# sndels/yuki

Measured on AMD Instinct MI355X. Metric: Mray/s (primary+secondary), Path integrator @1080p, higher is better.
Workload: dtype f32; 1 GPU; cfg3: city 40x20 displaced icospheres, 1,024,012 triangles, SAH BVH (max_shapes_in_node 1), Path 8 bounces, Stratified 8x8, 1920x1080; triangles=1024012, spp=64, max_depth=8, tiles=8160, partition=single GPU, frames_in_flight=2

## Files before the change

### include/yuki_hip.h

```cpp
#ifndef YUKI_HIP_H
#define YUKI_HIP_H
#include <stddef.h>
#include <stdint.h>

#ifdef __cplusplus
extern "C" {
#endif

#define YK_ABI_VERSION 1

typedef enum yk_status {
    YK_OK = 0,
    YK_ERR_INVALID_ARGUMENT = 1,
    YK_ERR_NO_DEVICE = 2,
    YK_ERR_DEVICE = 3,
    YK_ERR_OUT_OF_MEMORY = 4,
    YK_ERR_UNSUPPORTED = 5,
    YK_ERR_BVH_BUILD = 6,
    YK_ERR_CANCELLED = 7,
    YK_ERR_STACK_OVERFLOW = 8
} yk_status;


typedef struct yk_mesh_desc {
// ... 136 lines not shown
    uint32_t builder;
    uint32_t reason;
    uint32_t levels;
    uint32_t small_range;
    uint64_t small_ranges;
    double seconds_upload;
    double seconds_levels;
    double seconds_small;
    double seconds_layout;
    double seconds_copy_back;
} yk_bvh_build_info;

typedef struct yk_render_stats {
    uint64_t rays;
    uint64_t shadow_rays;
    uint64_t samples;
    double seconds_total;
    double seconds_trace;
    double seconds_shadow;
    double seconds_shade;
    uint32_t trace_launches, batches;
    uint32_t shadow_launches, reserved;
} yk_render_stats;

typedef struct yk_context yk_context;
typedef struct yk_scene yk_scene;

typedef int (*yk_cancel_fn)(void* user);

uint32_t yk_abi_version(void);
const char* yk_status_string(yk_status s);
yk_status yk_context_create(int device, yk_context** out);
void yk_context_destroy(yk_context* ctx);
yk_status yk_last_error(const yk_context* ctx, char* buf, size_t cap);
void* yk_context_stream(const yk_context* ctx);
yk_status yk_context_interrupt(yk_context* ctx);
yk_status yk_context_set_option(yk_context* ctx, const char* key, int64_t value);

yk_status yk_camera_init(const yk_camera_params* params, yk_camera* out);
size_t yk_film_tiles(uint16_t res_x, uint16_t res_y, uint16_t tile_dim, yk_tile* out, size_t cap);
yk_status yk_make_rect_light(const float light_to_world[16], const float light_to_world_inv[16], const float radiance[3],
                             const float size[2], yk_light_desc* out);
yk_status yk_make_spot_light(const float light_to_world[16], const float light_to_world_inv[16], const float intensity[3],
                             float total_width_degrees, float falloff_start_degrees, yk_light_desc* out);
yk_status yk_make_point_light(const float light_to_world[16], const float intensity[3], yk_light_desc* out);
yk_status yk_film_update_tiles(const yk_tile* tiles, size_t n_tiles, const float* tile_rgb, uint16_t res_x, uint16_t res_y,
                               float* film_rgb);

yk_status yk_scene_create(yk_context* ctx, const yk_scene_desc* desc, yk_scene** out);
yk_status yk_scene_create_device(yk_context* ctx, const yk_scene_desc* desc, void* stream, yk_scene** out);
yk_status yk_scene_update(yk_context* ctx, yk_scene* scene, const float* points, const float* normals);
yk_status yk_scene_update_device(yk_context* ctx, yk_scene* scene, const float* d_points, const float* d_normals, void* stream);
enum { YK_UPDATE_ROUTE_HOST = 0, YK_UPDATE_ROUTE_DEVICE = 1 };
typedef struct yk_scene_update_info {
    uint32_t n_updates;
    uint32_t route;
    uint32_t reason;
    uint32_t n_levels;
    uint64_t plan_bytes;
    double seconds_check, seconds_boxes, seconds_records, seconds_total;
} yk_scene_update_info;
yk_status yk_scene_get_update_info(const yk_scene* scene, yk_scene_update_info* out);
yk_status yk_bvh_refit(yk_bvh_node* nodes, size_t n_nodes, const uint32_t* shape_order, size_t n_shapes, const float* shape_bounds);
void yk_scene_destroy(yk_scene* scene);
yk_status yk_scene_get_info(const yk_scene* scene, yk_scene_info* out);
yk_status yk_scene_export_bvh(const yk_scene* scene, yk_bvh_node* nodes, uint32_t* shape_order);
yk_status yk_scene_get_build_info(const yk_scene* scene, yk_bvh_build_info* out);
enum { YK_LAYOUT_HOST = 0, YK_LAYOUT_DEVICE = 1 };
enum {
    YK_LAYOUT_REASON_NONE = 0,
    YK_LAYOUT_REASON_OUT_OF_MEMORY = 1,
    YK_LAYOUT_REASON_DEVICE_ERROR = 2,
    YK_LAYOUT_REASON_MULTI = 3
};
typedef struct yk_scene_layout_info {
    uint32_t layout;
    uint32_t reason;
    double seconds_upload;
    double seconds_layout;
    uint32_t tree_fetched;
    uint32_t root_ref, n_top, n_top_any, wide, wide_auto;
} yk_scene_layout_info;
yk_status yk_scene_get_layout_info(const yk_scene* scene, yk_scene_layout_info* out);
enum { YK_RECORDS_NODES = 0, YK_RECORDS_NODES4 = 1, YK_RECORDS_TOP = 2, YK_RECORDS_TOP_ANY = 3, YK_RECORDS_TRIS = 4, YK_RECORDS_PRIM_SHADE = 5, YK_RECORDS_PRIM_ATTR = 6 };
yk_status yk_scene_read_records(const yk_scene* scene, uint32_t which, void* out, size_t cap_bytes, size_t* n_bytes);
size_t yk_layout_top_order(const yk_bvh_node* nodes, size_t n, uint32_t cap, uint32_t* out_order);
size_t yk_layout_wide_slots(const yk_bvh_node* nodes, size_t n, uint32_t* out_slot_per_node);
size_t yk_bvh_partition_plan(const uint8_t* pass, size_t n, uint32_t* order);

yk_status yk_render_tiles(yk_context* ctx, const yk_scene* scene, const yk_camera* camera, const yk_sampler_desc* sampler,
                          const yk_integrator_desc* integrator, const yk_tile* tiles, size_t n_tiles, float* out_rgb,
                          yk_render_stats* stats, yk_cancel_fn cancel, void* user);
yk_status yk_render_tiles_device(yk_context* ctx, const yk_scene* scene, const yk_camera* camera,
                                 const yk_sampler_desc* sampler, const yk_integrator_desc* integrator, const yk_tile* tiles,
                                 size_t n_tiles, void* d_out_rgb, void* stream, yk_render_stats* stats, yk_cancel_fn cancel,
                                 void* user);
yk_status yk_render_tiles_accumulating(yk_context* ctx, const yk_scene* scene, const yk_camera* camera, const yk_sampler_desc* sampler,
                                       const yk_integrator_desc* integrator, const yk_tile* tiles, const uint16_t* tile_samples, size_t n_tiles,
                                       float* out_rgb, yk_render_stats* stats, yk_cancel_fn cancel, void* user);
yk_status yk_render_tiles_accumulating_device(yk_context* ctx, const yk_scene* scene, const yk_camera* camera, const yk_sampler_desc* sampler,
                                              const yk_integrator_desc* integrator, const yk_tile* tiles, const uint16_t* tile_samples,
                                              size_t n_tiles, void* d_out_rgb, void* stream, yk_render_stats* stats, yk_cancel_fn cancel,
                                              void* user);
yk_status yk_film_accumulate_tiles(const yk_tile* tiles, size_t n_tiles, const float* tile_rgb, uint16_t res_x, uint16_t res_y, float* film_rgb,
                                   uint32_t* tile_sample_counts);
yk_status yk_film_accumulate_tiles_device(yk_context* ctx, const yk_tile* tiles, size_t n_tiles, const void* d_tile_rgb, uint16_t res_x,
                                          uint16_t res_y, void* d_film_rgb, void* stream);
typedef struct yk_tile_list yk_tile_list;
yk_status yk_tile_list_create(yk_context* ctx, const yk_tile* tiles, const uint16_t* tile_samples, size_t n_tiles, yk_tile_list** out);
void yk_tile_list_destroy(yk_tile_list* list);
yk_status yk_render_tile_list_device(yk_context* ctx, const yk_scene* scene, const yk_camera* camera, const yk_sampler_desc* sampler,
                                     const yk_integrator_desc* integrator, const yk_tile_list* list, void* d_out_rgb, void* stream,
                                     yk_render_stats* stats, yk_cancel_fn cancel, void* user);
yk_status yk_film_update_tile_list_device(yk_context* ctx, const yk_tile_list* list, const void* d_tile_rgb, uint16_t res_x, uint16_t res_y,
                                          void* d_film_rgb, void* stream, int accumulate);
yk_status yk_render_tiles_accumulating_passes(yk_context* ctx, const yk_scene* scene, const yk_camera* camera, const yk_sampler_desc* sampler,
                                              const yk_integrator_desc* integrator, const yk_tile* tiles, const uint16_t* tile_samples,
                                              size_t n_tiles, uint32_t n_passes, float* out_rgb, yk_render_stats* stats, yk_cancel_fn cancel,
                                              void* user);
yk_status yk_render_tile_list_passes_device(yk_context* ctx, const yk_scene* scene, const yk_camera* camera, const yk_sampler_desc* sampler,
                                            const yk_integrator_desc* integrator, const yk_tile_list* list, uint32_t n_passes, void* d_out_rgb,
                                            void* stream, yk_render_stats* stats, yk_cancel_fn cancel, void* user);
yk_status yk_render_tile_list_samples_device(yk_context* ctx, const yk_scene* scene, const yk_camera* camera, const yk_sampler_desc* sampler,
                                             const yk_integrator_desc* integrator, const yk_tile_list* list, uint32_t first_sample,
                                             uint32_t n_passes, void* d_out_rgb, void* stream, yk_render_stats* stats, yk_cancel_fn cancel,
                                             void* user);
yk_status yk_film_accumulate_tile_list_passes_device(yk_context* ctx, const yk_tile_list* list, const void* d_passes_rgb, uint32_t n_passes,
                                                     uint16_t res_x, uint16_t res_y, void* d_film_rgb, void* stream);

yk_status yk_write_exr(const char* path, uint32_t width, uint32_t height, const float* rgb);
yk_status yk_write_pfm(const char* path, uint32_t width, uint32_t height, const float* rgb);

typedef enum yk_tone_map_kind { YK_TONE_MAP_RAW = 0, YK_TONE_MAP_FILMIC = 1, YK_TONE_MAP_HEATMAP = 2 } yk_tone_map_kind;
typedef enum yk_heatmap_channel { YK_HEATMAP_RED = 0, YK_HEATMAP_GREEN = 1, YK_HEATMAP_BLUE = 2, YK_HEATMAP_LUMINANCE = 3 } yk_heatmap_channel;
typedef struct yk_tone_map_desc {
    uint32_t kind;
    float exposure;
    uint32_t channel;
    uint32_t has_bounds;
    float bounds[2];
} yk_tone_map_desc;
yk_status yk_tone_map(yk_context* ctx, const yk_tone_map_desc* desc, const float* film_rgb, uint16_t res_x, uint16_t res_y,
                      uint16_t tile_dim, const uint32_t* samples, float* out_rgb, float* used_bounds);
yk_status yk_tone_map_device(yk_context* ctx, const yk_tone_map_desc* desc, const void* d_film_rgb, uint16_t res_x, uint16_t res_y,
                             uint16_t tile_dim, const uint32_t* samples, void* d_out_rgb, void* stream);
yk_status yk_film_min_max(yk_context* ctx, const float* film_rgb, uint16_t res_x, uint16_t res_y, uint32_t channel, float out_min_max[2]);

typedef struct yk_exposure_desc {
    uint32_t low_cut, high_cut;
    float ev_bias, min_ev, max_ev, adapt_up, adapt_down;
    uint16_t window[4];
} yk_exposure_desc;
typedef struct yk_exposure_state {
    float exposure, log2_adapted, log2_metered;
    uint32_t frames, counted, skipped, below, above;
} yk_exposure_state;
yk_status yk_film_histogram(yk_context* ctx, const float* film_rgb, uint16_t res_x, uint16_t res_y, uint16_t tile_dim, const uint32_t* samples,
                            const uint16_t window[4], uint32_t out_bins[256], uint32_t out_skipped_below_above[3]);
yk_status yk_exposure_meter(yk_context* ctx, const yk_exposure_desc* desc, const float* film_rgb, uint16_t res_x, uint16_t res_y, uint16_t tile_dim,
                            const uint32_t* samples, const yk_exposure_state* prev, yk_exposure_state* out);
yk_status yk_exposure_meter_device(yk_context* ctx, const yk_exposure_desc* desc, const void* d_film_rgb, uint16_t res_x, uint16_t res_y,
                                   uint16_t tile_dim, const uint32_t* samples, const void* d_prev, void* d_out_state, void* stream);
yk_status yk_tone_map_metered_device(yk_context* ctx, const yk_tone_map_desc* desc, const void* d_state, const void* d_film_rgb, uint16_t res_x,
                                     uint16_t res_y, uint16_t tile_dim, const uint32_t* samples, void* d_out_rgb, void* stream);

yk_status yk_render_tile(yk_context* ctx, const yk_scene* scene, const yk_camera* camera, const yk_sampler_desc* sampler,
                         const yk_integrator_desc* integrator, const yk_tile* tile, float* tile_pixels, uint64_t* out_rays);
yk_status yk_film_update_tiles_device(yk_context* ctx, const yk_tile* tiles, size_t n_tiles, const void* d_tile_rgb,
// ... 296 lines not shown
```

### yuki_amd/_ffi.py

```python
import ctypes as C
import os
import subprocess

from . import abi

_HERE = os.path.dirname(os.path.abspath(__file__))
LIB_PATH = os.environ.get("YK_LIB_PATH") or os.path.join(_HERE, "libyuki_hip.so")
_LIB = None

YK_OK = 0
STATUS_NAMES = {
    0: "YK_OK",
    1: "YK_ERR_INVALID_ARGUMENT",
    2: "YK_ERR_NO_DEVICE",
    3: "YK_ERR_DEVICE",
    4: "YK_ERR_OUT_OF_MEMORY",
    5: "YK_ERR_UNSUPPORTED",
    6: "YK_ERR_BVH_BUILD",
    7: "YK_ERR_CANCELLED",
    8: "YK_ERR_STACK_OVERFLOW",
}


class YukiError(RuntimeError):
# ... 6 lines not shown
    _fields_ = [
        ("n_nodes", C.c_uint64),
        ("n_interior", C.c_uint64),
        ("n_shapes", C.c_uint64),
        ("bounds_min", C.c_float * 3),
        ("bounds_max", C.c_float * 3),
        ("build_seconds", C.c_double),
        ("upload_seconds", C.c_double),
        ("device_bytes", C.c_uint64),
        ("max_leaf_shapes", C.c_uint32),
        ("tree_depth", C.c_uint32),
    ]


class BvhBuildInfo(C.Structure):
    _fields_ = [
        ("builder", C.c_uint32),
        ("reason", C.c_uint32),
        ("levels", C.c_uint32),
        ("small_range", C.c_uint32),
        ("small_ranges", C.c_uint64),
        ("seconds_upload", C.c_double),
        ("seconds_levels", C.c_double),
        ("seconds_small", C.c_double),
        ("seconds_layout", C.c_double),
        ("seconds_copy_back", C.c_double),
    ]


BVH_BUILDER_NAMES = {0: "host recursion", 1: "device", 2: "host levels"}
BVH_REASON_NAMES = {0: "", 1: "split method", 2: "non-finite bound", 3: "select_nth on a long range", 4: "too many nodes", 5: "out of device memory", 6: "device error"}


class RenderStats(C.Structure):
    _fields_ = [
        ("rays", C.c_uint64),
        ("shadow_rays", C.c_uint64),
        ("samples", C.c_uint64),
        ("seconds_total", C.c_double),
        ("seconds_trace", C.c_double),
        ("seconds_shadow", C.c_double),
        ("seconds_shade", C.c_double),
        ("trace_launches", C.c_uint32),
        ("batches", C.c_uint32),
        ("shadow_launches", C.c_uint32),
        ("reserved", C.c_uint32),
    ]


class CombinerInfo(C.Structure):
    _fields_ = [("submissions", C.c_uint64), ("tiles", C.c_uint64), ("requeued", C.c_uint64), ("largest_submission", C.c_uint32), ("lanes", C.c_uint32)]


CANCEL_FN = C.CFUNCTYPE(C.c_int, C.c_void_p)

vp = C.c_void_p
SYMBOLS = {
    "yk_abi_version": (C.c_uint32, []),
    "yk_status_string": (C.c_char_p, [C.c_int]),
    "yk_context_create": (C.c_int, [C.c_int, C.POINTER(vp)]),
    "yk_context_destroy": (None, [vp]),
    "yk_last_error": (C.c_int, [vp, C.c_char_p, C.c_size_t]),
    "yk_context_stream": (vp, [vp]),
    "yk_context_set_option": (C.c_int, [vp, C.c_char_p, C.c_int64]),
    "yk_camera_init": (C.c_int, [C.POINTER(abi.CameraParams), C.POINTER(abi.CameraMatrices)]),
    "yk_film_tiles": (C.c_size_t, [C.c_uint16, C.c_uint16, C.c_uint16, vp, C.c_size_t]),
    "yk_make_rect_light": (C.c_int, [abi.f32p, abi.f32p, abi.f32p, abi.f32p, C.POINTER(abi.LightDesc)]),
    "yk_make_spot_light": (C.c_int, [abi.f32p, abi.f32p, abi.f32p, C.c_float, C.c_float, C.POINTER(abi.LightDesc)]),
    "yk_make_point_light": (C.c_int, [abi.f32p, abi.f32p, C.POINTER(abi.LightDesc)]),
    "yk_film_update_tiles": (C.c_int, [vp, C.c_size_t, vp, C.c_uint16, C.c_uint16, vp]),
    "yk_scene_create": (C.c_int, [vp, C.POINTER(abi.SceneDesc), C.POINTER(vp)]),
    "yk_scene_create_device": (C.c_int, [vp, C.POINTER(abi.SceneDesc), vp, C.POINTER(vp)]),
    "yk_scene_update": (C.c_int, [vp, vp, vp, vp]),
    "yk_scene_update_device": (C.c_int, [vp, vp, vp, vp, vp]),
    "yk_scene_get_update_info": (C.c_int, [vp, C.POINTER(abi.SceneUpdateInfo)]),
    "yk_bvh_refit": (C.c_int, [vp, C.c_size_t, vp, C.c_size_t, vp]),
    "yk_scene_destroy": (None, [vp]),
    "yk_scene_get_info": (C.c_int, [vp, C.POINTER(SceneInfo)]),
    "yk_scene_export_bvh": (C.c_int, [vp, vp, vp]),
    "yk_scene_get_build_info": (C.c_int, [vp, C.POINTER(BvhBuildInfo)]),
    "yk_bvh_partition_plan": (C.c_size_t, [vp, C.c_size_t, vp]),
    "yk_scene_get_layout_info": (C.c_int, [vp, C.POINTER(abi.SceneLayoutInfo)]),
    "yk_scene_read_records": (C.c_int, [vp, C.c_uint32, vp, C.c_size_t, C.POINTER(C.c_size_t)]),
    "yk_layout_top_order": (C.c_size_t, [vp, C.c_size_t, C.c_uint32, vp]),
    "yk_layout_wide_slots": (C.c_size_t, [vp, C.c_size_t, vp]),
    "yk_render_tiles": (C.c_int, [vp, vp, C.POINTER(abi.CameraMatrices), C.POINTER(abi.SamplerDesc), C.POINTER(abi.IntegratorDesc), vp, C.c_size_t, vp, C.POINTER(RenderStats), vp, vp]),
    "yk_render_tiles_device": (C.c_int, [vp, vp, C.POINTER(abi.CameraMatrices), C.POINTER(abi.SamplerDesc), C.POINTER(abi.IntegratorDesc), vp, C.c_size_t, vp, vp, C.POINTER(RenderStats), vp, vp]),
    "yk_render_tile": (C.c_int, [vp, vp, C.POINTER(abi.CameraMatrices), C.POINTER(abi.SamplerDesc), C.POINTER(abi.IntegratorDesc), C.POINTER(abi.Tile), vp, C.POINTER(C.c_uint64)]),
    "yk_film_update_tiles_device": (C.c_int, [vp, vp, C.c_size_t, vp, C.c_uint16, C.c_uint16, vp, vp]),
    "yk_li": (C.c_int, [vp, vp, C.POINTER(abi.SamplerDesc), C.POINTER(abi.IntegratorDesc), C.c_size_t, vp, vp, vp, vp, C.c_uint32, vp, vp]),
    "yk_li_debug": (C.c_int, [vp, vp, C.POINTER(abi.SamplerDesc), C.POINTER(abi.IntegratorDesc), C.c_size_t, vp, vp, vp, vp, C.c_uint32, C.c_uint32, vp, vp, vp, vp]),
    "yk_trace_closest": (C.c_int, [vp, vp, C.c_size_t] + [vp] * 9),
    "yk_trace_any": (C.c_int, [vp, vp, C.c_size_t] + [vp] * 5),
    "yk_sampler_sequence": (C.c_int, [vp, C.POINTER(abi.SamplerDesc), C.c_uint16, C.c_uint16, C.c_uint32, vp, C.c_size_t, vp]),
    "yk_camera_rays": (C.c_int, [vp, C.POINTER(abi.CameraMatrices), C.POINTER(abi.SamplerDesc), C.POINTER(abi.Tile), C.c_uint32, vp, vp]),
    "yk_device_math": (C.c_int, [vp, C.c_int, C.c_size_t, vp, vp, vp]),
    "yk_host_math": (C.c_int, [C.c_int, C.c_size_t, vp, vp, vp]),
    "yk_bsdf_eval": (C.c_int, [vp, C.POINTER(abi.MaterialDesc), C.c_size_t] + [vp] * 6),
    "yk_bsdf_sample": (C.c_int, [vp, C.POINTER(abi.MaterialDesc), C.c_size_t] + [vp] * 6),
    "yk_light_sample": (C.c_int, [vp, C.POINTER(abi.LightDesc), C.c_int32, C.c_size_t] + [vp] * 4),
    "yk_sizeof": (C.c_size_t, [C.c_int]),
    "yk_load_ply": (C.c_int, [C.c_char_p, C.c_uint32, C.c_uint32, C.POINTER(vp)]),
    "yk_load_pbrt": (C.c_int, [C.c_char_p, C.c_uint32, C.c_uint32, C.POINTER(vp)]),
    "yk_load_mitsuba": (C.c_int, [C.c_char_p, C.c_uint32, C.c_uint32, C.POINTER(vp)]),
    "yk_load_scene": (C.c_int, [C.c_char_p, C.c_uint32, C.c_uint32, C.POINTER(vp)]),
    "yk_loaded_scene_get": (C.c_int, [vp, C.POINTER(abi.SceneDesc), C.POINTER(abi.CameraParams), C.POINTER(C.c_uint16)]),
    "yk_loaded_scene_destroy": (None, [vp]),
    "yk_loader_last_error": (C.c_char_p, []),
    "yk_image_texture_load": (C.c_int, [C.c_char_p, C.POINTER(abi.TextureDesc)]),
    "yk_image_texture_free": (None, [C.POINTER(abi.TextureDesc)]),
    "yk_render_tiles_accumulating": (C.c_int, [vp, vp, C.POINTER(abi.CameraMatrices), C.POINTER(abi.SamplerDesc), C.POINTER(abi.IntegratorDesc), vp, vp, C.c_size_t, vp, C.POINTER(RenderStats), vp, vp]),
    "yk_render_tiles_accumulating_device": (C.c_int, [vp, vp, C.POINTER(abi.CameraMatrices), C.POINTER(abi.SamplerDesc), C.POINTER(abi.IntegratorDesc), vp, vp, C.c_size_t, vp, vp, C.POINTER(RenderStats), vp, vp]),
    "yk_film_accumulate_tiles": (C.c_int, [vp, C.c_size_t, vp, C.c_uint16, C.c_uint16, vp, vp]),
    "yk_film_accumulate_tiles_device": (C.c_int, [vp, vp, C.c_size_t, vp, C.c_uint16, C.c_uint16, vp, vp]),
    "yk_tile_list_create": (C.c_int, [vp, vp, vp, C.c_size_t, C.POINTER(vp)]),
    "yk_tile_list_destroy": (None, [vp]),
    "yk_render_tile_list_device": (C.c_int, [vp, vp, C.POINTER(abi.CameraMatrices), C.POINTER(abi.SamplerDesc), C.POINTER(abi.IntegratorDesc), vp, vp, vp, C.POINTER(RenderStats), vp, vp]),
    "yk_film_update_tile_list_device": (C.c_int, [vp, vp, vp, C.c_uint16, C.c_uint16, vp, vp, C.c_int]),
    "yk_render_tiles_accumulating_passes": (C.c_int, [vp, vp, C.POINTER(abi.CameraMatrices), C.POINTER(abi.SamplerDesc), C.POINTER(abi.IntegratorDesc), vp, vp, C.c_size_t, C.c_uint32, vp, C.POINTER(RenderStats), vp, vp]),
    "yk_render_tile_list_samples_device": (C.c_int, [vp, vp, C.POINTER(abi.CameraMatrices), C.POINTER(abi.SamplerDesc), C.POINTER(abi.IntegratorDesc), vp, C.c_uint32, C.c_uint32, vp, vp, C.POINTER(RenderStats), vp, vp]),
    "yk_render_tile_list_passes_device": (C.c_int, [vp, vp, C.POINTER(abi.CameraMatrices), C.POINTER(abi.SamplerDesc), C.POINTER(abi.IntegratorDesc), vp, C.c_uint32, vp, vp, C.POINTER(RenderStats), vp, vp]),
    "yk_film_accumulate_tile_list_passes_device": (C.c_int, [vp, vp, vp, C.c_uint32, C.c_uint16, C.c_uint16, vp, vp]),
    "yk_write_exr": (C.c_int, [C.c_char_p, C.c_uint32, C.c_uint32, vp]),
    "yk_write_pfm": (C.c_int, [C.c_char_p, C.c_uint32, C.c_uint32, vp]),
    "yk_tone_map": (C.c_int, [vp, C.POINTER(abi.ToneMapDesc), vp, C.c_uint16, C.c_uint16, C.c_uint16, vp, vp, vp]),
    "yk_tone_map_device": (C.c_int, [vp, C.POINTER(abi.ToneMapDesc), vp, C.c_uint16, C.c_uint16, C.c_uint16, vp, vp, vp]),
    "yk_film_min_max": (C.c_int, [vp, vp, C.c_uint16, C.c_uint16, C.c_uint32, vp]),
    "yk_film_histogram": (C.c_int, [vp, vp, C.c_uint16, C.c_uint16, C.c_uint16, vp, vp, vp, vp]),
    "yk_exposure_meter": (C.c_int, [vp, C.POINTER(abi.ExposureDesc), vp, C.c_uint16, C.c_uint16, C.c_uint16, vp, C.POINTER(abi.ExposureState), C.POINTER(abi.ExposureState)]),
    "yk_exposure_meter_device": (C.c_int, [vp, C.POINTER(abi.ExposureDesc), vp, C.c_uint16, C.c_uint16, C.c_uint16, vp, vp, vp, vp]),
    "yk_tone_map_metered_device": (C.c_int, [vp, C.POINTER(abi.ToneMapDesc), vp, vp, C.c_uint16, C.c_uint16, C.c_uint16, vp, vp, vp]),
    "yk_scene_node_bounds": (C.c_size_t, [vp, C.c_int32, vp, C.c_size_t]),
    "yk_overlay_world_to_clip": (C.c_int, [C.POINTER(abi.CameraParams), vp, vp]),
    "yk_overlay_ray_lines": (C.c_int, [vp, C.c_size_t, vp]),
    "yk_overlay_draw": (C.c_int, [vp, vp, vp, C.c_size_t, vp, C.c_size_t, vp, C.c_uint16, C.c_uint16]),
    "yk_overlay_draw_device": (C.c_int, [vp, vp, vp, C.c_size_t, vp, C.c_size_t, vp, C.c_uint16, C.c_uint16, vp]),
    "yk_present_target_rect": (C.c_int, [C.c_uint16, C.c_uint16, C.c_uint16, C.c_uint16, C.POINTER(abi.PresentRect)]),
    "yk_present": (C.c_int, [vp, C.POINTER(abi.PresentDesc), vp, C.c_uint16, C.c_uint16, vp]),
    "yk_present_device": (C.c_int, [vp, C.POINTER(abi.PresentDesc), vp, C.c_uint16, C.c_uint16, vp, vp]),
    "yk_render_guides": (C.c_int, [vp, vp, C.POINTER(abi.CameraMatrices), C.c_uint16, C.c_uint16, vp]),
    "yk_render_guides_device": (C.c_int, [vp, vp, C.POINTER(abi.CameraMatrices), C.c_uint16, C.c_uint16, vp, vp]),
    "yk_denoise": (C.c_int, [vp, C.POINTER(abi.DenoiseDesc), vp, vp, C.c_uint16, C.c_uint16, C.c_uint16, vp, vp]),
    "yk_denoise_device": (C.c_int, [vp, C.POINTER(abi.DenoiseDesc), vp, vp, C.c_uint16, C.c_uint16, C.c_uint16, vp, vp, vp]),
    "yk_history_reproject": (C.c_int, [vp, C.POINTER(abi.TemporalDesc), vp, vp, C.POINTER(abi.CameraMatrices), vp, C.c_uint16, C.c_uint16, vp]),
    "yk_history_reproject_device": (C.c_int, [vp, C.POINTER(abi.TemporalDesc), vp, vp, C.POINTER(abi.CameraMatrices), vp, C.c_uint16, C.c_uint16, vp, vp]),
    "yk_history_blend": (C.c_int, [vp, C.POINTER(abi.TemporalDesc), vp, C.c_uint16, C.c_uint16, C.c_uint16, vp, vp, vp, vp]),
    "yk_history_blend_device": (C.c_int, [vp, C.POINTER(abi.TemporalDesc), vp, C.c_uint16, C.c_uint16, C.c_uint16, vp, vp, vp, vp, vp]),
    "yk_render_guides_ids": (C.c_int, [vp, vp, C.POINTER(abi.CameraMatrices), C.c_uint16, C.c_uint16, vp, vp]),
    "yk_render_guides_ids_device": (C.c_int, [vp, vp, C.POINTER(abi.CameraMatrices), C.c_uint16, C.c_uint16, vp, vp, vp]),
    "yk_surface_motion": (C.c_int, [vp, vp, vp, vp, vp, C.c_uint16, C.c_uint16, vp]),
    "yk_surface_motion_device": (C.c_int, [vp, vp, vp, vp, vp, C.c_uint16, C.c_uint16, vp, vp]),
    "yk_surface_albedo": (C.c_int, [vp, vp, vp, C.c_uint16, C.c_uint16, vp]),
    "yk_surface_albedo_device": (C.c_int, [vp, vp, vp, C.c_uint16, C.c_uint16, vp, vp]),
    "yk_albedo_mean": (C.c_int, [vp, vp, vp, C.c_uint16, C.c_uint16, C.c_uint32, vp]),
    "yk_albedo_mean_device": (C.c_int, [vp, vp, vp, C.c_uint16, C.c_uint16, C.c_uint32, vp, vp]),
    "yk_render_albedo_mean": (C.c_int, [vp, vp, C.POINTER(abi.CameraMatrices), C.c_uint16, C.c_uint16, C.c_uint32, vp]),
    "yk_render_albedo_mean_device": (C.c_int, [vp, vp, C.POINTER(abi.CameraMatrices), C.c_uint16, C.c_uint16, C.c_uint32, vp, vp]),
    "yk_denoise_albedo": (C.c_int, [vp, C.POINTER(abi.DenoiseDesc), vp, vp, vp, C.c_uint16, C.c_uint16, C.c_uint16, vp, vp]),
    "yk_denoise_albedo_device": (C.c_int, [vp, C.POINTER(abi.DenoiseDesc), vp, vp, vp, C.c_uint16, C.c_uint16, C.c_uint16, vp, vp, vp]),
    "yk_history_reproject_moved": (C.c_int, [vp, C.POINTER(abi.TemporalDesc), vp, vp, C.POINTER(abi.CameraMatrices), vp, vp, C.c_uint16, C.c_uint16, vp]),
    "yk_history_reproject_moved_device": (C.c_int, [vp, C.POINTER(abi.TemporalDesc), vp, vp, C.POINTER(abi.CameraMatrices), vp, vp, C.c_uint16, C.c_uint16, vp, vp]),
    "yk_moments_blend": (C.c_int, [vp, C.POINTER(abi.TemporalDesc), vp, C.c_uint16, C.c_uint16, C.c_uint16, vp, vp, vp]),
    "yk_moments_blend_device": (C.c_int, [vp, C.POINTER(abi.TemporalDesc), vp, C.c_uint16, C.c_uint16, C.c_uint16, vp, vp, vp, vp]),
    "yk_variance": (C.c_int, [vp, C.POINTER(abi.VarianceDesc), vp, vp, vp, vp, C.c_uint16, C.c_uint16, C.c_uint16, vp, vp]),
    "yk_variance_device": (C.c_int, [vp, C.POINTER(abi.VarianceDesc), vp, vp, vp, vp, C.c_uint16, C.c_uint16, C.c_uint16, vp, vp, vp]),
    "yk_denoise_variance": (C.c_int, [vp, C.POINTER(abi.VarianceDesc), vp, vp, vp, vp, C.c_uint16, C.c_uint16, C.c_uint16, vp, vp]),
# ... 79 lines not shown
```

### yuki_amd/abi.py

```python
import ctypes as C

import numpy as np

f32p = C.POINTER(C.c_float)
u32p = C.POINTER(C.c_uint32)
i32p = C.POINTER(C.c_int32)


class MeshDesc(C.Structure):
    _fields_ = [("has_normals", C.c_uint8), ("has_uvs", C.c_uint8), ("swaps_handedness", C.c_uint8), ("pad", C.c_uint8)]


class SphereDesc(C.Structure):
    _fields_ = [
        ("object_to_world", C.c_float * 16),
        ("world_to_object", C.c_float * 16),
        ("radius", C.c_float),
        ("material", C.c_int32),
    ]


class MaterialDesc(C.Structure):
    _fields_ = [("kind", C.c_uint32), ("a", C.c_float * 3), ("b", C.c_float * 3), ("c", C.c_float), ("flags", C.c_uint32), ("a_texture", C.c_uint32)]

# ... 156 lines not shown
    _fields_ = [
        ("bmin", C.c_float * 3),
        ("bmax", C.c_float * 3),
        ("a", C.c_uint32),
        ("count", C.c_uint16),
        ("axis", C.c_uint8),
        ("is_leaf", C.c_uint8),
    ]


class SceneLayoutInfo(C.Structure):

    _fields_ = [
        ("layout", C.c_uint32),
        ("reason", C.c_uint32),
        ("seconds_upload", C.c_double),
        ("seconds_layout", C.c_double),
        ("tree_fetched", C.c_uint32),
        ("root_ref", C.c_uint32),
        ("n_top", C.c_uint32),
        ("n_top_any", C.c_uint32),
        ("wide", C.c_uint32),
        ("wide_auto", C.c_uint32),
    ]


class SceneUpdateInfo(C.Structure):

    _fields_ = [
        ("n_updates", C.c_uint32),
        ("route", C.c_uint32),
        ("reason", C.c_uint32),
        ("n_levels", C.c_uint32),
        ("plan_bytes", C.c_uint64),
        ("seconds_check", C.c_double),
        ("seconds_boxes", C.c_double),
        ("seconds_records", C.c_double),
        ("seconds_total", C.c_double),
    ]


class TraceStats(C.Structure):
    _fields_ = [
        ("closest_rays", C.c_uint64),
        ("closest_node_tests", C.c_uint64),
        ("closest_shape_tests", C.c_uint64),
        ("shadow_rays", C.c_uint64),
        ("shadow_node_tests", C.c_uint64),
        ("shadow_shape_tests", C.c_uint64),
    ]


BVH_NODE_DTYPE = np.dtype(
    [("bmin", "<f4", 3), ("bmax", "<f4", 3), ("a", "<u4"), ("count", "<u2"), ("axis", "u1"), ("is_leaf", "u1")]
)
TILE_DTYPE = np.dtype([("x0", "<u2"), ("y0", "<u2"), ("x1", "<u2"), ("y1", "<u2")])
INTEGRATOR_RAY_DTYPE = np.dtype([("o", "<f4", 3), ("d", "<f4", 3), ("t_max", "<f4"), ("ray_type", "<u4")])
OVERLAY_LINE_DTYPE = np.dtype([("p0", "<f4", 3), ("p1", "<f4", 3), ("rgb", "<f4", 3)])
GUIDE_DTYPE = np.dtype([("ns", "<f4", 3), ("hit", "<f4"), ("p", "<f4", 3), ("t", "<f4")])
HISTORY_DTYPE = np.dtype([("rgb", "<f4", 3), ("n", "<f4")])
SURFACE_NONE = 0xFFFFFFFF
SURFACE_ID_DTYPE = np.dtype([("shape", "<u4"), ("b", "<f4", 3)])
MOTION_DTYPE = np.dtype([("p_prev", "<f4", 3), ("known", "<f4")])
ALBEDO_DTYPE = np.dtype([("a", "<f4", 3), ("known", "<f4")])
ALBEDO_FLOOR = 0.015625
ALBEDO_MEAN_MAX_S = 8
MOMENTS_DTYPE = np.dtype([("m1", "<f4"), ("m2", "<f4"), ("frames", "<f4"), ("n", "<f4")])
PIXEL_STATS_DTYPE = np.dtype([("mean", "<f4"), ("m2", "<f4"), ("n", "<u4"), ("drawn", "<u4")])

SPLIT_SAH, SPLIT_MIDDLE, SPLIT_EQUAL_COUNTS = 0, 1, 2
MAT_MATTE, MAT_GLASS, MAT_METAL, MAT_GLOSSY = 0, 1, 2, 3
LIGHT_POINT, LIGHT_SPOT, LIGHT_DISTANT, LIGHT_RECT = 0, 1, 2, 3
SAMPLER_UNIFORM, SAMPLER_STRATIFIED = 0, 1
INTEGRATOR_WHITTED, INTEGRATOR_PATH, INTEGRATOR_BVH_INTERSECTIONS, INTEGRATOR_GEOMETRY_NORMALS, INTEGRATOR_SHADING_NORMALS, INTEGRATOR_SHADING_UVS = 0, 1, 2, 3, 4, 5
RAY_DIRECT, RAY_REFLECTION, RAY_REFRACTION, RAY_NORMAL, RAY_SHADOW = 0, 1, 2, 3, 4
FOV_X, FOV_Y = 0, 1
TONE_MAP_RAW, TONE_MAP_FILMIC, TONE_MAP_HEATMAP = 0, 1, 2
HEATMAP_RED, HEATMAP_GREEN, HEATMAP_BLUE, HEATMAP_LUMINANCE = 0, 1, 2, 3
PRESENT_ENCODE_NONE, PRESENT_ENCODE_SHADER, PRESENT_ENCODE_SRGB = 0, 1, 2
PRESENT_RGBA8, PRESENT_RGB32F = 0, 1
LAYOUT_HOST, LAYOUT_DEVICE = 0, 1
UPDATE_ROUTE_HOST, UPDATE_ROUTE_DEVICE = 0, 1
LAYOUT_REASON_NONE, LAYOUT_REASON_OUT_OF_MEMORY, LAYOUT_REASON_DEVICE_ERROR, LAYOUT_REASON_MULTI = 0, 1, 2, 3
RECORDS_NODES, RECORDS_NODES4, RECORDS_TOP, RECORDS_TOP_ANY, RECORDS_TRIS, RECORDS_PRIM_SHADE, RECORDS_PRIM_ATTR = range(7)
RECORD_NAMES = ("nodes", "nodes4", "top", "top_any", "tris", "prim_shade", "prim_attr")


def ptr(a, ty):
    if a is None:
        return C.cast(None, ty)
    assert a.flags["C_CONTIGUOUS"]
    return a.ctypes.data_as(ty)


def f3(v):
    return (C.c_float * 3)(*[float(x) for x in v])


def f16(m):
    return (C.c_float * 16)(*[float(x) for x in np.asarray(m, dtype=np.float32).reshape(16)])
```

### yuki_amd/core.py

```python
import ctypes as C
from dataclasses import dataclass

import numpy as np

from . import _ffi, abi
from ._ffi import BvhBuildInfo, RenderStats, SceneInfo, YukiError, check, lib


def _p(a):
    return None if a is None else a.ctypes.data_as(C.c_void_p)


def _vp(a):
    return C.c_void_p(a) if a else None


def _film(film):
    film = np.ascontiguousarray(film, dtype=np.float32)
    if film.ndim != 3 or film.shape[2] != 3:
        raise ValueError("film is (h, w, 3)")
    return film, film.shape[1], film.shape[0]


def _scene_diagonal(scene):
# ... 896 lines not shown

    def reproject_history_moved_device(self, d_prev_history_ptr, d_prev_guides_ptr, prev_camera, d_guides_ptr, d_motion_ptr, res, params, d_out_history_ptr, stream=None):
        d = _temporal_desc(params)
        check(lib().yk_history_reproject_moved_device(self.h, C.byref(d), _vp(d_prev_history_ptr), _vp(d_prev_guides_ptr), C.byref(prev_camera.matrices), _vp(d_guides_ptr), _vp(d_motion_ptr), int(res[0]), int(res[1]), _vp(d_out_history_ptr), _vp(stream)), self.h)

    def blend_history_device(self, d_film_ptr, res, params, tile_dim, samples, d_history_ptr, d_out_history_ptr, d_out_rgb_ptr, stream=None):
        d = _temporal_desc(params)
        samples = _blend_samples(res, tile_dim, samples)
        check(lib().yk_history_blend_device(self.h, C.byref(d), _vp(d_film_ptr), int(res[0]), int(res[1]), int(tile_dim), _p(samples), _vp(d_history_ptr), _vp(d_out_history_ptr), _vp(d_out_rgb_ptr), _vp(stream)), self.h)

    def blend_moments_device(self, d_film_ptr, res, params, tile_dim, samples, d_moments_ptr, d_out_moments_ptr, stream=None):
        d = _temporal_desc(params)
        samples = _blend_samples(res, tile_dim, samples)
        check(lib().yk_moments_blend_device(self.h, C.byref(d), _vp(d_film_ptr), int(res[0]), int(res[1]), int(tile_dim), _p(samples), _vp(d_moments_ptr), _vp(d_out_moments_ptr), _vp(stream)), self.h)

    def variance_device(self, d_moments_ptr, d_film_ptr, d_guides_ptr, res, params, tile_dim, samples, d_out_ptr, stream=None, albedo=None):
        d = _variance_desc(params)
        samples = _blend_samples(res, tile_dim, samples)
        check(lib().yk_variance_device(self.h, C.byref(d), _vp(d_moments_ptr), _vp(d_film_ptr), _vp(d_guides_ptr), _vp(albedo), int(res[0]), int(res[1]), int(tile_dim), _p(samples), _vp(d_out_ptr), _vp(stream)), self.h)

    def denoise_variance_device(self, d_film_ptr, d_guides_ptr, d_variance_ptr, res, params, tile_dim, samples, d_out_ptr, stream=None, albedo=None):
        d = _variance_desc(params)
        samples = _blend_samples(res, tile_dim, samples)
        check(lib().yk_denoise_variance_device(self.h, C.byref(d), _vp(d_film_ptr), _vp(d_guides_ptr), _vp(d_variance_ptr), _vp(albedo), int(res[0]), int(res[1]), int(tile_dim), _p(samples), _vp(d_out_ptr), _vp(stream)), self.h)

    def adaptive_select_device(self, d_stats_ptr, res, params, pixel_list, stream=None):
        d = _adaptive_desc(params)
        n = C.c_uint32(0)
        check(lib().yk_adaptive_select_device(self.h, C.byref(d), _vp(d_stats_ptr), int(res[0]), int(res[1]), pixel_list.h, C.byref(n), _vp(stream)), self.h)
        pixel_list.n = n.value
        return n.value

    def adaptive_accumulate_device(self, pixel_list, d_passes_ptr, n_passes, res, d_film_sum_ptr, d_stats_ptr, stream=None):
        check(lib().yk_adaptive_accumulate_device(self.h, pixel_list.h, _vp(d_passes_ptr), int(n_passes), int(res[0]), int(res[1]), _vp(d_film_sum_ptr), _vp(d_stats_ptr), _vp(stream)), self.h)

    def adaptive_resolve_device(self, d_film_sum_ptr, d_stats_ptr, res, d_out_rgb_ptr, d_out_variance_ptr, stream=None):
        check(lib().yk_adaptive_resolve_device(self.h, _vp(d_film_sum_ptr), _vp(d_stats_ptr), int(res[0]), int(res[1]), _vp(d_out_rgb_ptr), _vp(d_out_variance_ptr), _vp(stream)), self.h)

    @property
    def stream_handle(self):
        return int(lib().yk_context_stream(self.h) or 0)

    def close(self):
        if getattr(self, "h", None):
            lib().yk_context_destroy(self.h)
            self.h = None

    def __del__(self):
        try:
            self.close()
        except Exception:
            pass


def _device_addresses(given, table, ctx, stream):
    address, tensors = {}, []
    for name, (dtypes, expected) in table.items():
        a = given.get(name)
        if a is None or isinstance(a, (int, np.integer)):
            address[name] = int(a) if a else None
            continue
        if not hasattr(a, "data_ptr"):
            raise ValueError(f"{name}: expected a torch tensor or a device address, got {type(a).__name__}")
        if str(a.dtype).replace("torch.", "") not in dtypes:
            raise ValueError(f"{name}: element type {a.dtype}, expected {' or '.join(dtypes)}")
        if not a.is_contiguous():
            raise ValueError(f"{name}: the tensor is not contiguous")
        if a.numel() != expected:
            raise ValueError(f"{name}: {a.numel()} elements, expected {expected}")
        tensors.append((name, a))
    for name, a in tensors:
        if not a.is_cuda or a.device.index != ctx.device:
            raise ValueError(f"{name}: the tensor is on {a.device}, not on the context's device {ctx.device}")
        address[name] = a.data_ptr() or None
    if stream is None and tensors:
        import torch

        torch.cuda.current_stream(tensors[0][1].device).synchronize()
    elif stream is not None and not isinstance(stream, int):
        stream = stream.cuda_stream
    return address, stream


class Scene:

    def __init__(self, ctx, scene_data):
        self.ctx = ctx
        self.data = scene_data
        d, self._keep = scene_data.desc(LightFactory)
        self.n_lights = int(d.n_lights)
        h = C.c_void_p()
        check(lib().yk_scene_create(ctx.h if ctx else None, C.byref(d), C.byref(h)), ctx.h if ctx else None)
        self.h = h
        self._keep = None

    DEVICE_ARRAYS = {
        "points": (abi.f32p, ("float32",), "v", 3),
        "normals": (abi.f32p, ("float32",), "v", 3),
        "uvs": (abi.f32p, ("float32",), "v", 2),
        "indices": (abi.u32p, ("uint32", "int32"), "t", 3),
        "tri_mesh": (abi.u32p, ("uint32", "int32"), "t", 1),
        "tri_material": (abi.i32p, ("int32",), "t", 1),
        "tri_area_light": (abi.i32p, ("int32",), "t", 1),
        "shape_order": (abi.u32p, ("uint32", "int32"), "s", 1),
    }

    @classmethod
    def from_device(cls, ctx, scene_data, arrays, stream=None):
        unknown = set(arrays) - set(cls.DEVICE_ARRAYS)
        if unknown:
            raise ValueError(f"unknown device arrays {sorted(unknown)}; the names are {sorted(cls.DEVICE_ARRAYS)}")
        counts = {"v": int(scene_data.points.shape[0]), "t": int(scene_data.indices.shape[0])}
        counts["s"] = counts["t"] + len(scene_data.spheres)
        address, stream = _device_addresses(arrays, {name: (dtypes, k * counts[per]) for name, (_, dtypes, per, k) in cls.DEVICE_ARRAYS.items()}, ctx, stream)
        self = cls.__new__(cls)
        self.ctx, self.data = ctx, scene_data
        d, keep = scene_data.desc(LightFactory)
        for name, (ptype, _, _, _) in cls.DEVICE_ARRAYS.items():
            setattr(d, name, C.cast(C.c_void_p(address[name]), ptype))
        self.n_lights = int(d.n_lights)
        h = C.c_void_p()
        check(lib().yk_scene_create_device(ctx.h, C.byref(d), _vp(stream), C.byref(h)), ctx.h)
        self.h = h
        del keep
        return self

    def close(self):
        if getattr(self, "h", None):
            lib().yk_scene_destroy(self.h)
            self.h = None

    def __del__(self):
        try:
            self.close()
        except Exception:
            pass

    def info(self):
        i = SceneInfo()
        check(lib().yk_scene_get_info(self.h, C.byref(i)))
        return i

    def build_info(self):
        i = BvhBuildInfo()
        check(lib().yk_scene_get_build_info(self.h, C.byref(i)))
        return i

    def layout_info(self):
        i = abi.SceneLayoutInfo()
        check(lib().yk_scene_get_layout_info(self.h, C.byref(i)))
        return i

    def update(self, points, normals=None, stream=None):
        nv = int(self.data.points.shape[0])
        given = {"points": points, "normals": normals}
        if all(a is None or isinstance(a, np.ndarray) or isinstance(a, (list, tuple)) for a in given.values()):
            host = {}
            for name, a in given.items():
                if a is None:
                    host[name] = None
                    continue
                a = np.ascontiguousarray(a, dtype=np.float32)
                if a.size != 3 * nv:
                    raise ValueError(f"{name}: {a.size} elements, expected {3 * nv}")
                host[name] = a.reshape(nv, 3)
            ctx_h = self.ctx.h if self.ctx else None
# ... 488 lines not shown
```

### yuki_amd/csrc/yk_context.cpp

```cpp
#include <hip/hip_runtime.h>

#include <algorithm>
#include <chrono>
#include <cstdio>
#include <cstdlib>
#include <cstring>
#include <mutex>
#include <string>
#include <vector>

#include "yk_internal.h"

extern "C" {

uint32_t yk_abi_version(void) { return YK_ABI_VERSION; }

const char* yk_status_string(yk_status s) {
    switch (s) {
        case YK_OK: return "ok";
        case YK_ERR_INVALID_ARGUMENT: return "invalid argument";
        case YK_ERR_NO_DEVICE: return "no HIP device";
        case YK_ERR_DEVICE: return "HIP error";
        case YK_ERR_OUT_OF_MEMORY: return "out of device memory";
        case YK_ERR_UNSUPPORTED: return "unsupported on the device path";
// ... 75 lines not shown
    if (ctx->ws[1].stream) (void)hipStreamDestroy(ctx->ws[1].stream);
    if (ctx->ev_in) (void)hipEventDestroy(ctx->ev_in);
    if (ctx->ev_out) (void)hipEventDestroy(ctx->ev_out);
    DevBuf* all[] = {&ctx->sample_buf, &ctx->pixel_xy, &ctx->pixel_aux, &ctx->tiles, &ctx->tile_off, &ctx->counters, &ctx->stats4, &ctx->hit4,
                     &ctx->tile_sample, &ctx->pixel_sample, &ctx->film_tiles, &ctx->film_tile_off, &ctx->film_pixel_xy};
    for (DevBuf* b : all) b->release();
    for (DevBuf& b : ctx->scratch) b.release();
    ctx->tonemap.partials.release();
    ctx->tonemap.bounds.release();
    ctx->tonemap.samples.release();
    ctx->overlay.ids.release();
    ctx->denoise.ping[0].release();
    ctx->denoise.ping[1].release();
    ctx->denoise.samples.release();
    ctx->temporal.samples.release();
    ctx->adaptive.rank.release();
    ctx->adaptive.tile_count.release();
    ctx->albedo_mean.ids_band.release();
    ctx->exposure.slot.release();
    ctx->exposure.samples.release();
    if (ctx->tonemap.staging) (void)hipHostFree(ctx->tonemap.staging);
    if (ctx->tonemap.staged) (void)hipEventDestroy(ctx->tonemap.staged);
    for (hipEvent_t e : ctx->ev_pool) (void)hipEventDestroy(e);
    if (ctx->cancel_stream) {
        (void)hipStreamSynchronize(ctx->cancel_stream);
        (void)hipStreamDestroy(ctx->cancel_stream);
    }
    if (ctx->cancel_host) (void)hipHostFree(ctx->cancel_host);
    (void)hipStreamDestroy(ctx->stream);
    delete ctx;
}

yk_status yk_last_error(const yk_context* ctx, char* buf, size_t cap) {
    if (!buf || cap == 0) return YK_ERR_INVALID_ARGUMENT;
    if (!ctx) {
        std::snprintf(buf, cap, "%s", host_last_error().c_str());
        host_last_error().clear();
        return YK_OK;
    }
    std::snprintf(buf, cap, "%s", ctx->last_error.c_str());
    return YK_OK;
}

void* yk_context_stream(const yk_context* ctx) { return ctx ? (void*)ctx->stream : nullptr; }

yk_status yk_context_set_option(yk_context* ctx, const char* key, int64_t value) {
    if (!ctx || !key) return YK_ERR_INVALID_ARGUMENT;
    YK_LOCK(ctx);
    std::string k(key);
    if (k == "batch_paths") {
        if (value < 64 || value > ((int64_t)1 << 29)) return YK_ERR_INVALID_ARGUMENT;
        ctx->batch_paths = value;
    } else if (k == "sample_buf_cap") {
        if (value < (1 << 20)) return YK_ERR_INVALID_ARGUMENT;
        ctx->sample_buf_cap = value;
    } else if (k == "streams") {
        if (value < 1 || value > 2) return YK_ERR_INVALID_ARGUMENT;
        ctx->streams = value;
    } else if (k == "packet_bounces") {
        if (value < 0) return YK_ERR_INVALID_ARGUMENT;
        ctx->packet_bounces = value;
    } else if (k == "packet_shadow_bounces") {
        if (value < 0) return YK_ERR_INVALID_ARGUMENT;
        ctx->packet_shadow_bounces = value;
    } else if (k == "shade_reorder") {
        ctx->shade_reorder = value != 0;
    } else if (k == "overlap_shadow") {
        ctx->overlap_shadow = value != 0;
    } else if (k == "top_nodes") {
        if (value < 0 || value > YK_TOP_MAX) return YK_ERR_INVALID_ARGUMENT;
        ctx->top_nodes = value;
    } else if (k == "wide_bvh") {
        if (value < 0 || value > 2) return YK_ERR_INVALID_ARGUMENT;
        ctx->wide_bvh = value;
    } else if (k == "bvh_builder") {
        if (value < 0 || value > 1) return YK_ERR_INVALID_ARGUMENT;
        ctx->bvh_builder = value;
    } else if (k == "bvh_small_range") {
        if (value < 0 || value > (1 << 20)) return YK_ERR_INVALID_ARGUMENT;
        ctx->bvh_small_range = value;
    } else if (k == "scene_layout") {
        if (value < 0 || value > 1) return YK_ERR_INVALID_ARGUMENT;
        ctx->scene_layout = value;
    } else if (k == "trace_stage_kernel") {
        if (value < 0 || value > 2) return YK_ERR_INVALID_ARGUMENT;
        ctx->trace_stage_kernel = value;
    } else if (k == "overlay_coop_min") {
        if (value < 1 || value > 65536) return YK_ERR_INVALID_ARGUMENT;
        ctx->overlay.coop_min = value;
    } else if (k == "denoise_lds_max_step") {
        if (value < 0 || value > 2) return YK_ERR_INVALID_ARGUMENT;
        ctx->denoise.lds_max_step = value;
    } else if (k == "albedo_mean_band_rows") {
        if (value < 0 || value > 65535) return YK_ERR_INVALID_ARGUMENT;
        ctx->albedo_mean.band_rows = value;
    } else if (k == "exposure_wave_combine") {
        ctx->exposure.wave_combine = value != 0;
    } else if (k == "update_top_block") {
        ctx->update_top_block = value != 0;
    } else if (k == "time_kernels") {
        ctx->time_kernels = value;
    } else {
        return YK_ERR_INVALID_ARGUMENT;
    }
    return YK_OK;
}

yk_status yk_camera_init(const yk_camera_params* params, yk_camera* out) { return camera_init(params, out); }

size_t yk_film_tiles(uint16_t res_x, uint16_t res_y, uint16_t tile_dim, yk_tile* out, size_t cap) try {
    std::vector<yk_tile> t = film_tiles(res_x, res_y, tile_dim);
    if (out)
        for (size_t i = 0; i < t.size() && i < cap; ++i) out[i] = t[i];
    return t.size();
} catch (const std::exception&) {
    return 0;
}

yk_status yk_make_rect_light(const float l2w[16], const float l2w_inv[16], const float radiance[3], const float size[2], yk_light_desc* out) {
    if (!l2w || !l2w_inv || !radiance || !size || !out) return YK_ERR_INVALID_ARGUMENT;
    std::memset(out, 0, sizeof(*out));
    Xf light_to_world = xf_from(l2w, l2w_inv);
    Xf sample_to_light = xf_mul(xf_scale(size[0], 1.0f, size[1]), xf_translation(-0.5f, 0.0f, -0.5f));
    Xf sample_to_world = xf_mul(light_to_world, sample_to_light);
    out->kind = YK_LIGHT_RECT;
    for (int k = 0; k < 3; ++k) out->i[k] = radiance[k];
    std::memcpy(out->sample_to_world, sample_to_world.m, 64);
    std::memcpy(out->sample_to_world_inv, sample_to_world.mi, 64);
    out->area = size[0] * size[1];
    return YK_OK;
}

yk_status yk_make_spot_light(const float l2w[16], const float l2w_inv[16], const float intensity[3], float total_width_degrees,
                             float falloff_start_degrees, yk_light_desc* out) {
    if (!l2w || !l2w_inv || !intensity || !out) return YK_ERR_INVALID_ARGUMENT;
    std::memset(out, 0, sizeof(*out));
    V3 p = xf_point(l2w, V3{0.0f, 0.0f, 0.0f});
    out->kind = YK_LIGHT_SPOT;
    out->p[0] = p.x;
    out->p[1] = p.y;
    out->p[2] = p.z;
    for (int k = 0; k < 3; ++k) out->i[k] = intensity[k];
    out->cos_total_width = det_cosf(total_width_degrees * (YK_PI / 180.0f));
    out->cos_falloff_start = det_cosf(falloff_start_degrees * (YK_PI / 180.0f));
    std::memcpy(out->world_to_light, l2w_inv, 64);
    return YK_OK;
}

yk_status yk_make_point_light(const float l2w[16], const float intensity[3], yk_light_desc* out) {
    if (!l2w || !intensity || !out) return YK_ERR_INVALID_ARGUMENT;
    std::memset(out, 0, sizeof(*out));
    V3 p = xf_point(l2w, V3{0.0f, 0.0f, 0.0f});
    out->kind = YK_LIGHT_POINT;
    out->p[0] = p.x;
    out->p[1] = p.y;
    out->p[2] = p.z;
    for (int k = 0; k < 3; ++k) out->i[k] = intensity[k];
    return YK_OK;
}

yk_status yk_film_update_tiles(const yk_tile* tiles, size_t n_tiles, const float* tile_rgb, uint16_t res_x, uint16_t res_y, float* film_rgb) {
    if (!tiles || !tile_rgb || !film_rgb) return YK_ERR_INVALID_ARGUMENT;
    size_t off = 0;
    for (size_t t = 0; t < n_tiles; ++t) {
        const yk_tile& tl = tiles[t];
        if (tl.x1 > res_x || tl.y1 > res_y || tl.x0 >= tl.x1 || tl.y0 >= tl.y1) return YK_ERR_INVALID_ARGUMENT;
// ... 57 lines not shown
```

### yuki_amd/csrc/yk_device.h

```cpp
#pragma once
#include <hip/hip_runtime.h>
#include <stdint.h>

#include "../../include/yuki_hip.h"
#include "yk_bsdf.h"
#include "yk_rng.h"

namespace yk {

struct DevNode {
    float4 q0, q1, q2;
    uint4 q3;
};
static_assert(sizeof(DevNode) == 64, "DevNode must be 64 bytes");

#define YK_VIS_STRIDE(nl) ((nl) <= 4u ? 4u : (nl))
#define YK_LEAF_BIT 0x80000000u
#define YK_REF_NONE 0xffffffffu
#define YK_AXIS_SHIFT 28
#define YK_AXIS_MASK (3u << YK_AXIS_SHIFT)
#define YK_REF_INDEX_MAX ((1u << YK_AXIS_SHIFT) - 1u)
#define YK_TOP_BIT 0x40000000u
#define YK_TOP_MAX 1023

struct DevNode4 {
    float4 q0, q1, q2, q3, q4, q5;
    uint4 q6, q7;
};
static_assert(sizeof(DevNode4) == 128, "DevNode4 must be 128 bytes");

struct DevLight {
    uint32_t kind;
    float p[3];
    float i[3];
    float cos_total_width, cos_falloff_start;
    float w2l[16];
    float s2w[16];
    float n[3];
    float area;
};

struct DevSphere {
    float o2w[16];
    float w2o[16];
    float radius;
    int material;
    unsigned swaps_handedness;
    unsigned pad;
};

#define YK_PRIM_LAST 1u
#define YK_PRIM_SPHERE 2u
#define YK_PRIM_KIND_SHIFT 4
#define YK_HIT_KIND_SHIFT 28
#define YK_HIT_PRIM_MASK 0x0fffffffu
#define YK_HIT_WORD(prim, pflags) ((int)((prim) | ((((pflags) >> YK_PRIM_KIND_SHIFT) & 7u) << YK_HIT_KIND_SHIFT)))

#define YK_MESH_NORMALS 1u
#define YK_MESH_UVS 2u
#define YK_MESH_SWAPS 4u

struct DevScene {
    const DevNode* nodes;
    const DevNode4* nodes4;
    const DevNode* top_nodes;
    uint32_t n_top;
    const DevNode* top_nodes_any;
    uint32_t n_top_any;
    const float4* tris;
    const uint4* prim_shade;
    const float4* prim_attr;
    const DevSphere* spheres;
    uint32_t n_triangles;
    uint32_t root_ref;
    float root_bmin[3], root_bmax[3];
    const uint32_t* indices;
    const float* points;
    const float* normals;
    const float* uvs;
    const uint32_t* tri_mesh;
    const int32_t* tri_material;
    const int32_t* tri_area_light;
    const uint32_t* mesh_flags;
    const Material* materials;
    const DevLight* lights;
    uint32_t n_lights;
    float background[3];
    const float4* texels;
    const uint4* tex_info;
};

struct DevCamera {
    float c2w[16];
    float r2c[16];
};

struct PathBuffers {
    float4* rayO;
    float4* rayD;
    float4* thru;
    uint4* rngs;
};

#define YK_CTRL_WORDS 1024
#define YK_CTRL_ERR 3
#define YK_CTRL_CANCELLED 2
#define YK_CTRL_CAM_O (YK_CTRL_WORDS + 32)
#define YK_CTRL_ALLOC_WORDS (YK_CTRL_WORDS + 64)
#define YK_CTRL_HEADS 8
#define YK_CTRL_STRIDE 8
#define YK_CTRL_BOUNCE(b) (8 + YK_CTRL_STRIDE * (b))
#define YK_CTRL_SHQ 1
#define YK_CTRL_SHQ2 2
#define YK_CTRL_HEAD 3
#define YK_CTRL_MAX_DEPTH ((YK_CTRL_WORDS - 8) / YK_CTRL_STRIDE - 1)

struct CancelRef {
    const unsigned* host;
    unsigned* dev;
};
#define YK_HEAD_POISON 0xC0000000u

__device__ __forceinline__ bool cancel_raised(const CancelRef& c) { return c.dev && *c.dev != 0u; }
__device__ __forceinline__ bool cancel_relay(const CancelRef& c, unsigned* head) {
    if (!c.host || __hip_atomic_load(c.host, __ATOMIC_RELAXED, __HIP_MEMORY_SCOPE_SYSTEM) == 0u) return false;
    atomicOr(c.dev, 1u);
    atomicMax(head, YK_HEAD_POISON);
    return true;
}

struct RenderParams {
    SamplerCfg sampler;
    uint32_t max_depth;
    uint32_t has_clamp;
    float clamp;
    uint32_t integrator;
    uint32_t spe;
    uint32_t sample_base;
    CancelRef cancel;
};

__device__ __forceinline__ void split_sample_id(uint32_t sid, uint32_t spe, uint32_t& entry, uint32_t& k) {
    if ((spe & (spe - 1u)) == 0u) {
        entry = sid >> (31u - (uint32_t)__clz((int)spe));
        k = sid & (spe - 1u);
    } else {
        entry = sid / spe;
        k = sid % spe;
    }
}

}
```

### yuki_amd/csrc/yk_geom.h

```cpp
#pragma once
#include "yk_device.h"

namespace yk {

struct RayTri {
    int kx, ky, kz;
    float sx, sy, sz;
};
YK_HD RayTri ray_tri_setup(V3 d) {
    RayTri r;
    r.kz = max_dimension(vabs(d));
    r.kx = r.kz < 2 ? r.kz + 1 : 0;
    r.ky = r.kx < 2 ? r.kx + 1 : 0;
    float dx = comp(d, r.kx), dy = comp(d, r.ky), dz = comp(d, r.kz);
    r.sx = -dx / dz;
    r.sy = -dy / dz;
    r.sz = 1.0f / dz;
    return r;
}

struct TriHit {
    float t, b0, b1, b2;
};

// ... 155 lines not shown
    } else {
        float inv_uv_det = 1.0f / uv_det;
        dpdu = (dp02 * duv12y - dp12 * duv02y) * inv_uv_det;
        dpdv = ((-dp02) * duv12x + dp12 * duv02x) * inv_uv_det;
    }
    (void)dpdv;
    Surface s;
    s.p = p0 * h.b0 + p1 * h.b1 + p2 * h.b2;
    s.u = u0x * h.b0 + u1x * h.b1 + u2x * h.b2;
    s.v = u0y * h.b0 + u1y * h.b1 + u2y * h.b2;
    V3 n = normalize(cross(dp02, dp12));
    if (mflags & YK_MESH_SWAPS) n = -n;
    s.n = n;
    s.ns = n;
    s.dpdus = dpdu;
    if (mflags & YK_MESH_NORMALS) {
        V3 n0 = at.n0, n1 = at.n1, n2 = at.n2;
        V3 ns;
        V3 nn = normalize(n0 * h.b0 + n1 * h.b1 + n2 * h.b2);
        if (len_sqr(nn) > 0.0f)
            ns = normalize(nn);
        else
            ns = s.n;
        V3 ss = normalize(dpdu);
        V3 ts = cross(ss, ns);
        if (len_sqr(ts) > 0.0f) {
            ts = normalize(ts);
            ss = cross(ts, ns);
        } else {
            coordinate_system(ns, ss, ts);
        }
        s.ns = normalize(cross(ss, ts));
        s.n = faceforward_n(s.n, s.ns);
        s.dpdus = ss;
    }
    s.material = 0;
    s.area_light = -1;
    return s;
}

YK_HD Surface make_surface_core(const DevScene& sc, V3 p0, V3 p1, V3 p2, uint32_t i0, uint32_t i1, uint32_t i2, uint32_t mflags, const TriHit& h) {
    TriAttr at;
    at.u0x = at.u0y = at.u1x = at.u1y = at.u2x = at.u2y = 0.0f;
    at.n0 = at.n1 = at.n2 = V3{0.0f, 0.0f, 0.0f};
    if (mflags & YK_MESH_UVS) {
        at.u0x = sc.uvs[2 * i0]; at.u0y = sc.uvs[2 * i0 + 1];
        at.u1x = sc.uvs[2 * i1]; at.u1y = sc.uvs[2 * i1 + 1];
        at.u2x = sc.uvs[2 * i2]; at.u2y = sc.uvs[2 * i2 + 1];
    }
    if (mflags & YK_MESH_NORMALS) {
        at.n0 = ld3(sc.normals, i0);
        at.n1 = ld3(sc.normals, i1);
        at.n2 = ld3(sc.normals, i2);
    }
    return make_surface_vals(p0, p1, p2, at, mflags, h);
}

YK_HD Surface make_surface(const DevScene& sc, uint32_t tri, const TriHit& h) {
    uint32_t i0 = sc.indices[3 * tri], i1 = sc.indices[3 * tri + 1], i2 = sc.indices[3 * tri + 2];
    Surface s = make_surface_core(sc, ld3(sc.points, i0), ld3(sc.points, i1), ld3(sc.points, i2), i0, i1, i2, sc.mesh_flags[sc.tri_mesh[tri]], h);
    s.material = sc.tri_material[tri];
    s.area_light = sc.tri_area_light[tri];
    return s;
}

YK_HD Surface hit_surface(const DevScene& sc, uint32_t shape, V3 o, V3 d) {
    if (shape >= sc.n_triangles) {
        const DevSphere& sp = sc.spheres[shape - sc.n_triangles];
        V3 ro, rd;
        float t = 0.0f;
        sphere_hit_t(sp, o, d, __builtin_inff(), t, ro, rd);
        return make_surface_sphere(sp, ro, rd, t, d, sc.texels != nullptr);
    }
    uint32_t i0 = sc.indices[3 * shape], i1 = sc.indices[3 * shape + 1], i2 = sc.indices[3 * shape + 2];
    RayTri rt = ray_tri_setup(d);
    TriHit th = TriHit{0.0f, 0.0f, 0.0f, 0.0f};
    tri_intersect(o, rt, __builtin_inff(), ld3(sc.points, i0), ld3(sc.points, i1), ld3(sc.points, i2), th);
    Surface s = make_surface(sc, shape, th);
    s.wo = -d;
    return s;
}

YK_HD Surface hit_surface_prim(const DevScene& sc, uint32_t prim, V3 o, V3 d, bool want_uv, float* t_out, uint4* id_out) {
    const float4 v0 = sc.tris[3 * prim], v1 = sc.tris[3 * prim + 1], v2 = sc.tris[3 * prim + 2];
    const uint4 ps = sc.prim_shade[prim];
    const uint32_t src = __float_as_uint(v1.w);
    if (__float_as_uint(v2.w) & YK_PRIM_SPHERE) {
        const DevSphere& sp = sc.spheres[src - sc.n_triangles];
        V3 ro, rd;
        float t = 0.0f;
        sphere_hit_t(sp, o, d, __builtin_inff(), t, ro, rd);
        if (t_out) *t_out = t;
        if (id_out) *id_out = make_uint4(src, 0u, 0u, 0u);
        return make_surface_sphere(sp, ro, rd, t, d, want_uv);
    }
    TriAttr at;
    at.u0x = at.u0y = at.u1x = at.u1y = at.u2x = at.u2y = 0.0f;
    at.n0 = at.n1 = at.n2 = V3{0.0f, 0.0f, 0.0f};
    if (sc.prim_attr && (ps.w & (YK_MESH_NORMALS | YK_MESH_UVS))) {
        const float4 a0 = sc.prim_attr[4 * (size_t)prim], a1 = sc.prim_attr[4 * (size_t)prim + 1], a2 = sc.prim_attr[4 * (size_t)prim + 2], a3 = sc.prim_attr[4 * (size_t)prim + 3];
        at.n0 = V3{a0.x, a0.y, a0.z};
        at.n1 = V3{a1.x, a1.y, a1.z};
        at.n2 = V3{a2.x, a2.y, a2.z};
        at.u0x = a0.w; at.u0y = a1.w;
        at.u1x = a2.w; at.u1y = a3.x;
        at.u2x = a3.y; at.u2y = a3.z;
    }
    RayTri rt = ray_tri_setup(d);
    TriHit th = TriHit{0.0f, 0.0f, 0.0f, 0.0f};
    const V3 p0 = V3{v0.x, v0.y, v0.z}, p1 = V3{v1.x, v1.y, v1.z}, p2 = V3{v2.x, v2.y, v2.z};
    tri_intersect(o, rt, __builtin_inff(), p0, p1, p2, th);
    if (t_out) *t_out = th.t;
    if (id_out) *id_out = make_uint4(src, __float_as_uint(th.b0), __float_as_uint(th.b1), __float_as_uint(th.b2));
    Surface s = sc.prim_attr ? make_surface_vals(p0, p1, p2, at, ps.w & 7u, th) : make_surface_core(sc, p0, p1, p2, ps.x, ps.y, ps.z, ps.w & 7u, th);
    s.material = (int)(ps.w >> 6);
    s.area_light = (int)__float_as_uint(v0.w);
    s.wo = -d;
    return s;
}
YK_HD Surface hit_surface_prim(const DevScene& sc, uint32_t prim, V3 o, V3 d, bool want_uv, float* t_out) { return hit_surface_prim(sc, prim, o, d, want_uv, t_out, nullptr); }
YK_HD Surface hit_surface_prim(const DevScene& sc, uint32_t prim, V3 o, V3 d, bool want_uv) { return hit_surface_prim(sc, prim, o, d, want_uv, nullptr, nullptr); }
YK_HD Surface hit_surface_prim(const DevScene& sc, uint32_t prim, V3 o, V3 d) { return hit_surface_prim(sc, prim, o, d, sc.texels != nullptr, nullptr, nullptr); }

YK_HD RGB texture_eval(const DevScene& sc, unsigned tex, float u, float v) {
    const uint4 info = sc.tex_info[tex];
    float sx = u - truncf(u);
    if (sx < 0.0f) sx = 1.0f + sx;
    float sy = v - truncf(v);
    if (sy < 0.0f) sy = 1.0f + sy;
    sy = 1.0f - sy;
    float fx = sx * (float)info.y - 0.5f;
    float fy = sy * (float)info.z - 0.5f;
    unsigned ix = fx > 0.0f ? (unsigned)fminf(fx, 4.0e9f) : 0u;
    unsigned iy = fy > 0.0f ? (unsigned)fminf(fy, 4.0e9f) : 0u;
    size_t idx = (size_t)iy * info.y + ix;
    const size_t last = (size_t)info.y * info.z - 1;
    if (idx > last) idx = last;
    float4 t = sc.texels[(size_t)info.x + idx];
    return RGB{t.x, t.y, t.z};
}

YK_HD V3 spawn_origin(V3 p, V3 n, V3 d) {
    V3 offset = n * 0.001f;
    return dot(d, n) > 0.0f ? p + offset : p - offset;
}

struct LightSample {
    V3 l;
    RGB li;
    float pdf;
    bool has_vis;
    V3 p1;
    int area_light;
};

YK_HD LightSample sample_light(const DevLight& L, int index, V3 sp, float ux, float uy) {
    LightSample s;
    s.has_vis = true;
    s.area_light = -1;
    s.pdf = 1.0f;
    V3 lp = V3{L.p[0], L.p[1], L.p[2]};
    RGB li = RGB{L.i[0], L.i[1], L.i[2]};
    if (L.kind == YK_LIGHT_POINT) {
        V3 to_light = lp - sp;
        float dist_sqr = len_sqr(to_light);
        s.li = li / dist_sqr;
        float dist = sqrtf(dist_sqr);
        s.l = to_light / dist;
        s.p1 = lp;
    } else if (L.kind == YK_LIGHT_SPOT) {
        V3 to_light = lp - sp;
        float dist_sqr = len_sqr(to_light);
        float dist = sqrtf(dist_sqr);
        s.l = to_light / dist;
        V3 dir_local = normalize(xf_vector(L.w2l, -s.l));
        float ct = dir_local.z;
        float falloff;
        if (ct < L.cos_total_width)
            falloff = 0.0f;
        else if (ct > L.cos_falloff_start)
            falloff = 1.0f;
        else {
            float delta = (ct - L.cos_total_width) / (L.cos_falloff_start - L.cos_total_width);
            falloff = (delta * delta) * (delta * delta);
        }
        s.li = li * falloff / dist_sqr;
        if (is_black(s.li)) s.has_vis = false;
        s.p1 = lp;
    } else if (L.kind == YK_LIGHT_DISTANT) {
        s.li = li;
        s.l = lp;
        s.p1 = sp + lp * 10000.0f;
    } else {
        V3 p = xf_point(L.s2w, V3{ux, 0.0f, uy});
        V3 n = V3{L.n[0], L.n[1], L.n[2]};
        V3 wi = normalize(p - sp);
        float ndw = dot_nv(n, -wi);
// ... 11 lines not shown
```

### yuki_amd/csrc/yk_internal.h

```cpp
#pragma once
#include <hip/hip_runtime.h>

#include <algorithm>
#include <atomic>
#include <chrono>
#include <memory>
#include <mutex>
#include <string>
#include <vector>

#include "yk_device.h"
#include "yk_host.h"
#include "yk_kernels.h"
#include "yk_scene_input.h"
#include "yk_scene_records.h"

using namespace yk;

struct DevBuf {
    void* p = nullptr;
    size_t bytes = 0;
    hipError_t ensure(size_t want) {
        if (want <= bytes) return hipSuccess;
        if (p) (void)hipFree(p);
        p = nullptr;
        bytes = 0;
        hipError_t e = hipMalloc(&p, want);
        if (e == hipSuccess) bytes = want;
        return e;
    }
    void release() {
        if (p) (void)hipFree(p);
        p = nullptr;
        bytes = 0;
    }
    template <class T> T* as() const { return reinterpret_cast<T*>(p); }
};
static inline hipError_t put_host_array(DevBuf& buf, const void* src, size_t bytes) {
    hipError_t e = buf.ensure(std::max<size_t>(bytes, 16));
    if (e == hipSuccess && bytes) e = hipMemcpy(buf.p, src, bytes, hipMemcpyHostToDevice);
    return e;
}

static inline uint32_t layout_reason_of(hipError_t e) {
    (void)hipGetLastError();
    return e == hipErrorOutOfMemory ? YK_LAYOUT_REASON_OUT_OF_MEMORY : YK_LAYOUT_REASON_DEVICE_ERROR;
}

struct DevScratch {
    std::vector<void*> all;
    hipError_t err = hipSuccess;
    ~DevScratch() {
        for (void* p : all) (void)hipFree(p);
    }
    template <class T> bool get(T*& out, size_t count) {
        void* p = nullptr;
        if ((err = hipMalloc(&p, std::max<size_t>(count * sizeof(T), 16))) != hipSuccess) {
            (void)hipGetLastError();
            return false;
        }
        all.push_back(p);
        out = reinterpret_cast<T*>(p);
        return true;
    }
    template <class T> void give(T* p, size_t count, DevBuf& to) {
        all.erase(std::find(all.begin(), all.end(), (void*)p));
        to.release();
        to.p = p;
        to.bytes = std::max<size_t>(count * sizeof(T), 16);
    }
};

#define YK_ALBEDO_MEAN_SCRATCH ((size_t)64 << 20)
#define YK_BVH_SMALL_RANGE 32

struct yk_context {
    int device = 0;
    hipStream_t stream = nullptr;
    std::string last_error;
    int n_cu = 256;
    int64_t batch_paths = 128 << 20;
    int64_t packet_bounces = 1;
    int64_t packet_shadow_bounces = 1;
    int64_t shade_reorder = 1;
    int64_t overlap_shadow = 1;
    int64_t wide_bvh = 2;
    int64_t top_nodes = YK_TOP_MAX;
    int64_t bvh_builder = 0;
    int64_t bvh_small_range = YK_BVH_SMALL_RANGE;
    int64_t scene_layout = 0;
    int64_t trace_stage_kernel = 0;
    int64_t update_top_block = 1;
    int64_t sample_buf_cap = (int64_t)64 << 30;
    int64_t time_kernels = 1;
    int64_t streams = 2;
    struct WorkSet {
        DevBuf path[2][4];
        DevBuf hit, pend, shO, shD, shC, vis, shq, shO2, shD2, shq2, ctrl, spill, spill_side;
        size_t cap_paths = 0;
        unsigned cap_lights = 0, cap_area = 0, cap_delta = 0;
        hipStream_t stream = nullptr;
        hipStream_t side = nullptr;
        hipEvent_t done = nullptr, ev_shade = nullptr, ev_acc = nullptr;
        hipEvent_t ev_batch = nullptr;
    } ws[2];
    DevBuf sample_buf, pixel_xy, pixel_aux, tiles, tile_off, counters, stats4, hit4;
    DevBuf tile_sample, pixel_sample;
    DevBuf film_tiles, film_tile_off, film_pixel_xy;
    DevBuf scratch[8];
    std::vector<hipEvent_t> ev_pool;
    hipEvent_t ev_in = nullptr, ev_out = nullptr;
    unsigned* cancel_host = nullptr;
    const unsigned* cancel_host_dev = nullptr;
    hipStream_t cancel_stream = nullptr;
    bool want_cancel_stream = false;
    std::atomic<bool> cancel_raised{false};
    struct ToneMapState {
        DevBuf partials, bounds, samples;
        uint32_t* staging = nullptr;
        size_t staging_words = 0;
        hipEvent_t staged = nullptr;
    } tonemap;
    struct DenoiseState {
        DevBuf ping[2];
        DevBuf samples;
        int64_t lds_max_step = 2;
    } denoise;
    struct TemporalState {
        DevBuf samples;
    } temporal;
    struct OverlayState {
        DevBuf ids;
        int64_t coop_min = 32;
    } overlay;
    struct AdaptiveState {
        DevBuf rank;
        DevBuf tile_count;
    } adaptive;
    struct AlbedoMeanState {
        DevBuf ids_band;
        int64_t band_rows = 0;
    } albedo_mean;
    struct ExposureState {
        DevBuf slot;
        DevBuf samples;
        int64_t wave_combine = 1;
    } exposure;
    std::recursive_mutex mu;
};

typedef yk_context::WorkSet WorkSet;
static const uint32_t YK_WIDE_MAX_PATHS = 6u << 20;

struct DeviceTree {
    DevBuf nodes, depth, order;
    uint32_t n_nodes = 0, n_shapes = 0;
    uint32_t root_words[8] = {};
    void release() {
        nodes.release();
        depth.release();
        order.release();
    }
};

struct yk_scene {
    int device = -1;
    std::shared_ptr<const HostBvh> bvh;
    std::shared_ptr<HostBvh> bvh_lazy;
    DevBuf tree_nodes, tree_order;
    mutable std::mutex tree_mu;
    mutable std::atomic<uint32_t> tree_fetched{1};
    yk_scene_layout_info layout = {};
    size_t record_bytes[7] = {};
    uint32_t n_triangles = 0, n_spheres = 0, n_lights = 0, n_delta_lights = 0;
    uint32_t n_materials = 0, n_meshes = 0, n_textures = 0;
    bool wide_auto = false;
    yk_scene_info info;
    yk_bvh_build_info build_info;
    mutable std::vector<uint8_t> shape_kind;
    std::vector<uint8_t> lazy_mat_kind, lazy_sphere_kind;
    bool shape_kind_lazy = false;
    mutable std::once_flag kind_once;
    mutable std::atomic<uint32_t> kind_fetched{1};
    DevBuf nodes, nodes4, top_nodes, top_nodes_any, tris, prim_shade, prim_attr, indices, points, normals, uvs, tri_mesh, tri_material, tri_area_light, mesh_flags, materials, lights, spheres, texels, tex_info;
    DevScene dev;
    bool on_device = false;
    struct UpdateState {
        uint32_t n_vertices = 0;
        bool has_normals = false, has_uvs = false;
        LayoutOptions opt;
        std::vector<float> sphere_bounds;
        std::vector<uint8_t> mat_kind;
        std::vector<uint32_t> host_indices;
        bool planned = false;
        DevBuf depth, list, sphere_b, mat_kind_d, words;
        std::vector<uint32_t> level_off;
        yk_scene_update_info info = {};
    } upd;
    struct ShadingTables {
        std::vector<uint32_t> indices, tri_mesh, mesh_flags;
        std::vector<int32_t> tri_material;
        std::vector<float> uvs;
        std::vector<Material> materials;
        std::vector<DevSphere> spheres;
        std::vector<float4> texels;
        std::vector<uint4> tex_info;
    } host_shading;
};

static inline DevScene dev_scene_for(const yk_scene* scene, uint64_t n) {
    DevScene ds = scene->dev;
    if (scene->wide_auto && n > YK_WIDE_MAX_PATHS) ds.nodes4 = nullptr;
    return ds;
}

struct yk_tile_list {
    int device = -1;
    std::vector<yk_tile> tiles;
    std::vector<uint16_t> samples;
    std::vector<uint32_t> off;
    DevBuf pixel_xy, pixel_sample;
};

struct yk_pixel_list {
    yk_context* ctx = nullptr;
    uint32_t res_x = 0, res_y = 0;
    uint32_t n = 0;
    uint32_t passes = 0;
    uint32_t sample_end = 0;
    DevBuf pixel_xy, pixel_sample;
};

inline std::string& host_last_error() {
    static thread_local std::string msg;
    return msg;
}
static inline yk_status fail(yk_context* ctx, yk_status st, const std::string& msg) {
    if (ctx)
        ctx->last_error = msg;
    else
        host_last_error() = msg;
    return st;
}

#define YK_LOCK(ctx) std::lock_guard<std::recursive_mutex> yk_lock_((ctx)->mu)
#define HIP_TRY(ctx, expr)                                                                                           \
    do {                                                                                                             \
        hipError_t _e = (expr);                                                                                      \
        if (_e != hipSuccess) {                                                                                      \
            return fail(ctx, _e == hipErrorOutOfMemory ? YK_ERR_OUT_OF_MEMORY : YK_ERR_DEVICE,                       \
                        std::string(#expr) + ": " + hipGetErrorString(_e));                                          \
        }                                                                                                            \
    } while (0)

#define YK_CATCH(ctx)                                                                                         \
    catch (const std::bad_alloc&) { return fail(ctx, YK_ERR_OUT_OF_MEMORY, "host allocation failed"); }      \
    catch (const std::exception& e) { return fail(ctx, YK_ERR_INVALID_ARGUMENT, std::string("exception: ") + e.what()); }


struct SceneImage;
struct SceneBuild {
    bool device_builder, device_layout;
    uint32_t layout_reason;
};
yk_status yk_build_scene_image(yk_context* opt_ctx, const yk_scene_desc* d, std::shared_ptr<SceneImage>& out, const SceneBuild& what);
yk_status yk_upload_scene_image(yk_context* ctx, const std::shared_ptr<SceneImage>& img, yk_scene** out);

const HostBvh* scene_host_tree(const yk_scene* scene);

const std::vector<uint8_t>* scene_shape_kind(const yk_scene* scene);

static inline double now_seconds() {
    return std::chrono::duration<double>(std::chrono::steady_clock::now().time_since_epoch()).count();
}

bool build_bvh_device(yk_context* ctx, const std::vector<ShapeBounds>& bounds, uint32_t max_shapes_in_node, uint32_t split_method, uint32_t small_range, HostBvh& out, yk_bvh_build_info& bi,
                      DeviceTree* keep = nullptr);
bool build_bvh_device(yk_context* ctx, const ShapeBounds* h_bounds, const float* d_bounds, size_t n_bounds, uint32_t max_shapes_in_node, uint32_t split_method, uint32_t small_range, HostBvh& out,
                      yk_bvh_build_info& bi, DeviceTree* keep);
bool build_bvh_levels(const std::vector<ShapeBounds>& bounds, uint32_t max_shapes_in_node, uint32_t split_method, uint32_t small_range, HostBvh& out, yk_bvh_build_info& bi);

uint32_t layout_scene_device(yk_context* ctx, yk_scene* s, const DeviceTree& tree, const uint32_t* d_user_order, const uint8_t* d_mat_kind, bool has_attr, uint32_t tree_depth, bool* order_applied);

uint32_t update_scene_device(yk_context* ctx, yk_scene* s, const float* d_points, const float* d_normals, bool* not_finite);

hipError_t enqueue_geometry_checks(hipStream_t st, const inp::Geometry& g, const uint8_t* d_light_kind, const uint32_t* d_order, uint32_t n_shapes, uint32_t* d_seen, inp::CheckWords* d_words);
hipError_t enqueue_shape_bounds(hipStream_t st, const float* d_points, const uint32_t* d_indices, const uint32_t* d_order, const float* d_sphere_bounds, uint32_t n_triangles, uint32_t n_shapes, float* d_sb,
                                inp::CheckWords* d_words);

yk_status stage_sample_table(yk_context* ctx, hipStream_t st, const uint32_t* samples, uint16_t res_x, uint16_t res_y, uint16_t tile_dim, DevBuf& dst);
inline yk_status stage_samples(yk_context* ctx, hipStream_t st, const uint32_t* samples, uint16_t res_x, uint16_t res_y, uint16_t tile_dim, DevBuf& dst, const uint32_t** d_samples) {
    *d_samples = nullptr;
    if (!samples) return YK_OK;
    yk_status s = stage_sample_table(ctx, st, samples, res_x, res_y, tile_dim, dst);
    if (s == YK_OK) *d_samples = dst.as<const uint32_t>();
    return s;
}

yk_status adaptive_select_into(yk_context* ctx, hipStream_t st, const yk_adaptive_desc* desc, const void* d_stats, yk_pixel_list* list, uint32_t* out_n);

void set_record_layout(yk_scene* s, size_t n_interior, size_t n_wide, size_t n_top, size_t n_top_any, size_t n_shapes, bool has_attr, uint32_t root_ref, bool wide_auto);
hipError_t upload_host_tree(const HostBvh& bvh, DeviceTree& tree);
void adopt_device_tree(yk_scene* s, DeviceTree& tree, const std::shared_ptr<HostBvh>& lazy);
Material make_material(const yk_material_desc& m);
DevLight make_light(const yk_light_desc& l);

#define YK_COUNTER_BYTES 256
unsigned* error_block(yk_context* ctx);
CancelRef cancel_ref(yk_context* ctx);
yk_status ensure_work_buffers(yk_context* ctx, WorkSet& ws, size_t paths, unsigned n_lights, unsigned n_delta_lights);
yk_status ensure_spill(yk_context* ctx, WorkSet& ws);
unsigned trace_grid(const yk_context* ctx);
PathBuffers path_buffers(WorkSet& ws, int which);
yk_status make_params(yk_context* ctx, const yk_sampler_desc* smp, const yk_integrator_desc* integ, RenderParams& prm);

struct KernelTimer {
    yk_context* ctx;
    bool on;
    std::vector<std::pair<int, int>> spans[3];
    size_t used = 0;
    int begin(hipStream_t s) {
        if (!on) return -1;
        if (used + 2 > ctx->ev_pool.size()) {
            size_t old = ctx->ev_pool.size();
            ctx->ev_pool.resize(old + 256);
            for (size_t i = old; i < ctx->ev_pool.size(); ++i) (void)hipEventCreate(&ctx->ev_pool[i]);
        }
        int a = (int)used;
        used += 2;
        (void)hipEventRecord(ctx->ev_pool[a], s);
        return a;
    }
    void end(int a, int cls, hipStream_t s) {
        if (a < 0) return;
        (void)hipEventRecord(ctx->ev_pool[a + 1], s);
        spans[cls].push_back(std::make_pair(a, a + 1));
    }
    double total(int cls) {
        double ms = 0.0;
        for (auto& sp : spans[cls]) {
            float t = 0.0f;
            if (hipEventElapsedTime(&t, ctx->ev_pool[sp.first], ctx->ev_pool[sp.second]) == hipSuccess) ms += t;
        }
        return ms * 1e-3;
    }
};

bool packet_kernel_traces_bounce(const yk_context* ctx, const yk_scene* scene, unsigned b);
void run_bounces(yk_context* ctx, WorkSet& ws, hipStream_t st, const yk_scene* scene, const RenderParams& prm, const uint32_t* pixel_xy,
                 const uint32_t* sample_index_tab, float4* sample_buf, KernelTimer& kt, unsigned long long* counters, bool coherent,
                 uint32_t n_paths, uint32_t sid_base, bool lean_camera_bounce, uint32_t* n_shadow_launches = nullptr);
```

### yuki_amd/csrc/yk_scene.cpp

```cpp
#include <hip/hip_runtime.h>

#include <algorithm>
#include <array>
#include <chrono>
#include <cstdio>
#include <cstdlib>
#include <cstring>
#include <mutex>
#include <string>
#include <vector>

#include "yk_internal.h"
#include "yk_scene_layout.h"
#include "yk_scene_update.h"

template <class T> static yk_status upload(yk_context* ctx, DevBuf& buf, const T* src, size_t count) {
    size_t bytes = std::max<size_t>(count * sizeof(T), 16);
    HIP_TRY(ctx, buf.ensure(bytes));
    if (count) HIP_TRY(ctx, hipMemcpy(buf.p, src, count * sizeof(T), hipMemcpyHostToDevice));
    return YK_OK;
}

typedef std::unique_ptr<yk_scene, void (*)(yk_scene*)> ScenePtr;

static void set_scene_counts(yk_scene* s, const yk_scene_desc* d) {
    s->n_triangles = d->n_triangles;
    s->n_spheres = d->n_spheres;
    s->n_lights = d->n_lights;
    s->n_materials = d->n_materials;
    s->n_meshes = d->n_meshes;
    s->n_textures = d->n_textures;
    for (uint32_t l = 0; l < d->n_lights; ++l) s->n_delta_lights += d->lights[l].kind != YK_LIGHT_RECT ? 1u : 0u;
}

Material make_material(const yk_material_desc& m) {
    Material r;
    std::memset(&r, 0, sizeof(r));
    for (int k = 0; k < 3; ++k) {
        r.a[k] = m.a[k];
        r.b[k] = m.b[k];
    }
    const bool remap = (m.flags & YK_MAT_FLAG_REMAP) != 0;
    const bool textured = m.kind == YK_MAT_MATTE && (m.flags & YK_MAT_FLAG_TEXTURED_A) != 0;
    r.tex = textured ? m.a_texture + 1u : 0u;
    switch (m.kind) {
        case YK_MAT_MATTE: {
            if (!textured && m.a[0] == 0.0f && m.a[1] == 0.0f && m.a[2] == 0.0f) {
                r.kind = MK_BLACK;
            } else if (m.c == 0.0f) {
                r.kind = MK_LAMBERT;
            } else {
                r.kind = MK_OREN_NAYAR;
                float sigma2 = m.c * m.c;
                r.c = 1.0f - (sigma2 / (2.0f * (sigma2 + 0.33f)));
                r.d = 0.45f * sigma2 / (sigma2 + 0.09f);
            }
            break;
        }
        case YK_MAT_GLASS:
            r.kind = MK_GLASS;
            r.c = m.c;
            break;
        case YK_MAT_METAL: {
            r.kind = MK_METAL;
            float roughness = remap ? roughness_to_alpha(m.c) : m.c;
            r.c = rmax(roughness, 0.001f);
            break;
        }
        default: {
            r.kind = MK_GLOSSY;
            float roughness = remap ? roughness_to_alpha(m.c) : m.c;
            r.c = rmax(roughness * roughness, 0.001f);
            break;
        }
    }
    return r;
}

DevLight make_light(const yk_light_desc& l) {
    DevLight d;
    std::memset(&d, 0, sizeof(d));
    d.kind = l.kind;
    for (int k = 0; k < 3; ++k) {
        d.p[k] = l.p[k];
        d.i[k] = l.i[k];
    }
    d.cos_total_width = l.cos_total_width;
    d.cos_falloff_start = l.cos_falloff_start;
    std::memcpy(d.w2l, l.world_to_light, 64);
    std::memcpy(d.s2w, l.sample_to_world, 64);
    V3 n = xf_normal(l.sample_to_world_inv, V3{0.0f, -1.0f, 0.0f});
    d.n[0] = n.x;
    d.n[1] = n.y;
    d.n[2] = n.z;
    d.area = l.area;
    return d;
}

static std::array<DevBuf*, 22> scene_buffers(yk_scene* s) {
    return {&s->nodes,    &s->nodes4,       &s->top_nodes,      &s->top_nodes_any, &s->tris,      &s->prim_shade, &s->prim_attr, &s->indices, &s->points,  &s->normals,    &s->uvs,
            &s->tri_mesh, &s->tri_material, &s->tri_area_light, &s->mesh_flags,    &s->materials, &s->lights,     &s->spheres,   &s->texels,  &s->tex_info, &s->tree_nodes, &s->tree_order};
}
static const DevBuf& record_buffer(const yk_scene* s, uint32_t which) { return *scene_buffers(const_cast<yk_scene*>(s))[which]; }

void set_record_layout(yk_scene* s, size_t n_interior, size_t n_wide, size_t n_top, size_t n_top_any, size_t n_shapes, bool has_attr, uint32_t root_ref, bool wide_auto) {
    yk_scene_layout_info& li = s->layout;
    li.root_ref = root_ref;
    li.n_top = (uint32_t)n_top;
    li.n_top_any = (uint32_t)n_top_any;
    li.wide = n_wide ? 1u : 0u;
    li.wide_auto = wide_auto ? 1u : 0u;
    s->record_bytes[YK_RECORDS_NODES] = std::max<size_t>(n_interior, 1) * sizeof(DevNode);
    s->record_bytes[YK_RECORDS_NODES4] = n_wide * sizeof(DevNode4);
    s->record_bytes[YK_RECORDS_TOP] = n_top * sizeof(DevNode);
    s->record_bytes[YK_RECORDS_TOP_ANY] = n_top_any * sizeof(DevNode);
    s->record_bytes[YK_RECORDS_TRIS] = 3 * n_shapes * sizeof(float4);
    s->record_bytes[YK_RECORDS_PRIM_SHADE] = n_shapes * sizeof(uint4);
    s->record_bytes[YK_RECORDS_PRIM_ATTR] = has_attr ? 4 * n_shapes * sizeof(float4) : 0;
}

struct SceneImage {
    std::shared_ptr<const HostBvh> bvh;
    std::shared_ptr<HostBvh> bvh_mut;
    bool device_layout = false, tree_on_device = false, order_applied = false;
    uint32_t layout_reason = 0;
    DeviceTree dtree;
    ~SceneImage() { dtree.release(); }
    const yk_scene_desc* d = nullptr;
    yk_scene_info info;
    yk_bvh_build_info build_info;
    LayoutOptions opt;
    bool has_device_records = false;
    SceneRecords rec;
    std::vector<float4> texels;
    std::vector<uint4> tex_info;
    std::vector<uint32_t> mesh_flags, tri_mesh;
    std::vector<uint8_t> mat_kind;
    std::vector<int32_t> tri_al;
    std::vector<uint8_t> shape_kind;
    std::vector<Material> mats;
    std::vector<DevSphere> spheres;
    std::vector<DevLight> lights;
};

static yk_status check_description(yk_context* ctx, const yk_scene_desc* d, bool arrays_on_host = true) {
    if ((uint64_t)d->n_triangles + d->n_spheres == 0) return fail(ctx, YK_ERR_INVALID_ARGUMENT, "empty scene");
    if (d->n_triangles && (!d->points || !d->indices)) return fail(ctx, YK_ERR_INVALID_ARGUMENT, "missing geometry arrays");
    if (d->max_shapes_in_node == 0 || d->max_shapes_in_node > 65535u || d->split_method > 2) return fail(ctx, YK_ERR_INVALID_ARGUMENT, "bad BVH settings");
    for (uint32_t i = 0; arrays_on_host && i < d->n_triangles; ++i) {
        for (int k = 0; k < 3; ++k)
            if (d->indices[3 * i + k] >= d->n_vertices) return fail(ctx, YK_ERR_INVALID_ARGUMENT, "vertex index out of range");
        if (d->tri_mesh && d->tri_mesh[i] >= d->n_meshes) return fail(ctx, YK_ERR_INVALID_ARGUMENT, "mesh index out of range");
        if (d->tri_material && (d->tri_material[i] < 0 || (uint32_t)d->tri_material[i] >= d->n_materials))
            return fail(ctx, YK_ERR_INVALID_ARGUMENT, "material index out of range");
        if (d->tri_area_light && d->tri_area_light[i] >= (int32_t)d->n_lights) return fail(ctx, YK_ERR_INVALID_ARGUMENT, "light index out of range");
    }
    if ((d->n_spheres && !d->spheres) || (d->n_materials && !d->materials) || (d->n_lights && !d->lights) || (d->n_meshes && !d->meshes))
        return fail(ctx, YK_ERR_INVALID_ARGUMENT, "a count is non-zero but its array is NULL");
    if (d->tri_area_light && arrays_on_host)
        for (uint32_t i = 0; i < d->n_triangles; ++i) {
            const int32_t al = d->tri_area_light[i];
            if (al < -1 || (al >= 0 && d->lights[al].kind != YK_LIGHT_RECT)) return fail(ctx, YK_ERR_INVALID_ARGUMENT, "tri_area_light must be -1 or index a rectangular light");
        }
    for (uint32_t k = 0; k < d->n_spheres; ++k)
        if (d->spheres[k].material < 0 || (uint32_t)d->spheres[k].material >= d->n_materials) return fail(ctx, YK_ERR_INVALID_ARGUMENT, "sphere material out of range");
    for (uint32_t m = 0; m < d->n_materials; ++m)
        if ((d->materials[m].flags & YK_MAT_FLAG_TEXTURED_A) && d->materials[m].kind == YK_MAT_MATTE && d->materials[m].a_texture >= d->n_textures)
            return fail(ctx, YK_ERR_INVALID_ARGUMENT, "material texture index out of range");
    if (d->n_materials >= (1u << 26)) return fail(ctx, YK_ERR_UNSUPPORTED, "more than 2^26 materials");
    for (uint32_t t = 0; t < d->n_textures; ++t)
        if (!d->textures || !d->textures[t].rgb || d->textures[t].width == 0 || d->textures[t].height == 0 || d->textures[t].width >= (1u << 24) ||
            d->textures[t].height >= (1u << 24))
            return fail(ctx, YK_ERR_INVALID_ARGUMENT, "bad texture");
    if (d->n_triangles && (!d->tri_material || d->n_materials == 0 || d->n_meshes == 0))
        return fail(ctx, YK_ERR_INVALID_ARGUMENT, "triangles need materials and meshes");
    for (uint32_t m = 0; m < d->n_meshes; ++m) {
        if (d->meshes[m].has_normals && !d->normals) return fail(ctx, YK_ERR_INVALID_ARGUMENT, "mesh has_normals without a normals array");
        if (d->meshes[m].has_uvs && !d->uvs) return fail(ctx, YK_ERR_INVALID_ARGUMENT, "mesh has_uvs without a uvs array");
    }
    return YK_OK;
}

static ShapeBounds sphere_bound(const yk_sphere_desc& sp) {
    const float r = sp.radius;
    const float lo[3] = {-r, -r, -r}, hi[3] = {r, r, r};
    const float big = 3.40282347e+38f;
    ShapeBounds b = {{big, big, big}, {-big, -big, -big}};
    const int corner[8][3] = {{0, 0, 0}, {1, 0, 0}, {0, 1, 0}, {0, 0, 1}, {1, 1, 0}, {1, 0, 1}, {0, 1, 1}, {1, 1, 1}};
    for (int c = 0; c < 8; ++c) {
        V3 q = xf_point(sp.object_to_world, V3{corner[c][0] ? hi[0] : lo[0], corner[c][1] ? hi[1] : lo[1], corner[c][2] ? hi[2] : lo[2]});
        const float qq[3] = {q.x, q.y, q.z};
        for (int k = 0; k < 3; ++k) {
            b.bmin[k] = rmin(b.bmin[k], qq[k]);
            b.bmax[k] = rmax(b.bmax[k], qq[k]);
        }
    }
    return b;
}
static yk_status shape_bounds(yk_context* ctx, const yk_scene_desc* d, std::vector<ShapeBounds>& sb) {
    sb.assign((size_t)d->n_triangles + d->n_spheres, ShapeBounds());
    for (uint32_t i = 0; i < d->n_triangles; ++i) {
// ... 59 lines not shown
    }
}

static yk_status small_tables(yk_context* ctx, const yk_scene_desc* d, SceneImage* s) {
    s->mats.resize(std::max<uint32_t>(d->n_materials, 1));
    s->mat_kind.assign(s->mats.size(), 0u);
    for (uint32_t m = 0; m < d->n_materials; ++m) {
        s->mats[m] = make_material(d->materials[m]);
        s->mat_kind[m] = (uint8_t)(s->mats[m].kind & 7u);
    }
    s->mesh_flags.assign(std::max<uint32_t>(d->n_meshes, 1), 0);
    for (uint32_t m = 0; m < d->n_meshes; ++m)
        s->mesh_flags[m] = (d->meshes[m].has_normals ? YK_MESH_NORMALS : 0u) | (d->meshes[m].has_uvs ? YK_MESH_UVS : 0u) | (d->meshes[m].swaps_handedness ? YK_MESH_SWAPS : 0u);
    s->spheres.resize(std::max<uint32_t>(d->n_spheres, 1));
    for (uint32_t k = 0; k < d->n_spheres; ++k) {
        DevSphere& o = s->spheres[k];
        std::memcpy(o.o2w, d->spheres[k].object_to_world, 64);
        std::memcpy(o.w2o, d->spheres[k].world_to_object, 64);
        o.radius = d->spheres[k].radius;
        o.material = d->spheres[k].material;
        const float* m = o.o2w;
        float det = m[0] * (m[5] * m[10] - m[6] * m[9]) - m[1] * (m[4] * m[10] - m[6] * m[8]) + m[2] * (m[4] * m[9] - m[5] * m[8]);
        o.swaps_handedness = det < 0.0f ? 1u : 0u;
        o.pad = 0;
    }
    s->lights.resize(std::max<uint32_t>(d->n_lights, 1));
    for (uint32_t l = 0; l < d->n_lights; ++l) s->lights[l] = make_light(d->lights[l]);
    for (uint32_t t = 0; t < d->n_textures; ++t) {
        const yk_texture_desc& td = d->textures[t];
        s->tex_info.push_back(make_uint4((unsigned)s->texels.size(), td.width, td.height, 0u));
        const size_t n = (size_t)td.width * td.height;
        if (s->texels.size() + n > 0xffffffffull) return fail(ctx, YK_ERR_UNSUPPORTED, "more than 2^32 texels");
        for (size_t k = 0; k < n; ++k) s->texels.push_back(make_float4(td.rgb[3 * k], td.rgb[3 * k + 1], td.rgb[3 * k + 2], 0.0f));
    }
    return YK_OK;
}
static yk_status host_tables(yk_context* ctx, const yk_scene_desc* d, SceneImage* s) {
    yk_status st = small_tables(ctx, d, s);
    if (st != YK_OK) return st;
    s->shape_kind.resize(s->info.n_shapes);
    for (uint32_t i = 0; i < d->n_triangles; ++i) s->shape_kind[i] = s->mat_kind[d->tri_material[i]];
    for (uint32_t k = 0; k < d->n_spheres; ++k) s->shape_kind[(size_t)d->n_triangles + k] = s->mat_kind[d->spheres[k].material];
    s->tri_mesh.assign(d->n_triangles, 0);
    if (d->tri_mesh) std::memcpy(s->tri_mesh.data(), d->tri_mesh, sizeof(uint32_t) * d->n_triangles);
    s->tri_al.assign(d->n_triangles, -1);
    if (d->tri_area_light) std::memcpy(s->tri_al.data(), d->tri_area_light, sizeof(int32_t) * d->n_triangles);
    return YK_OK;
}

static void layout_image_host(SceneImage* s) {
    const yk_scene_desc* d = s->d;
    std::vector<int32_t> sphere_material(d->n_spheres);
    for (uint32_t k = 0; k < d->n_spheres; ++k) sphere_material[k] = d->spheres[k].material;
    HostLayoutInput in;
    in.bvh = s->bvh.get();
    in.n_interior = s->info.n_interior;
    in.indices = d->indices;
    in.points = d->points;
    in.normals = d->normals;
    in.uvs = d->uvs;
    in.tri_material = d->tri_material;
    in.tri_area_light = s->tri_al.data();
    in.tri_mesh = s->tri_mesh.data();
    in.mesh_flags = s->mesh_flags.data();
    in.n_triangles = d->n_triangles;
    in.sphere_material = sphere_material.data();
    in.mat_kind = s->mat_kind.data();
    in.opt = s->opt;
    s->rec = layout_records_host(in);
}

yk_status yk_build_scene_image(yk_context* ctx, const yk_scene_desc* d, std::shared_ptr<SceneImage>& out, const SceneBuild& what) try {
    if (!d) return fail(ctx, YK_ERR_INVALID_ARGUMENT, "null scene description");
    out.reset();
    yk_status st = check_description(ctx, d);
    if (st != YK_OK) return st;

    std::shared_ptr<SceneImage> img = std::make_shared<SceneImage>();
    SceneImage* s = img.get();
    s->bvh = s->bvh_mut = std::make_shared<HostBvh>();
    s->d = d;
    s->device_layout = ctx && what.device_layout;
    s->layout_reason = ctx ? what.layout_reason : 0u;
    if (ctx) s->opt = LayoutOptions{ctx->top_nodes, ctx->wide_bvh};
    std::memset(&s->info, 0, sizeof(s->info));

    std::vector<ShapeBounds> sb;
    if ((st = shape_bounds(ctx, d, sb)) != YK_OK || (st = build_tree(ctx, d, sb, what.device_builder, s)) != YK_OK) return st;
    fill_scene_info(s);
    if (ctx) {
        if (s->info.n_nodes > YK_REF_INDEX_MAX || s->info.n_shapes > YK_REF_INDEX_MAX) return fail(ctx, YK_ERR_UNSUPPORTED, "more than 2^28 BVH nodes or shapes");
        if ((st = host_tables(ctx, d, s)) != YK_OK) return st;
        if (!s->device_layout) layout_image_host(s);
        s->has_device_records = true;
    }
    out = img;
    return YK_OK;
} YK_CATCH(ctx)

static yk_status fetch_tree(int device, const DevBuf& d_nodes, const DevBuf& d_order, uint32_t n_nodes, uint32_t n_shapes, HostBvh& out) {
    if (!d_nodes.p || !d_order.p || !out.nodes.empty()) return YK_OK;
    (void)hipSetDevice(device);
    std::vector<yk_bvh_node> nodes(n_nodes);
    std::vector<uint32_t> order(n_shapes);
    if (hipMemcpy(nodes.data(), d_nodes.p, (size_t)n_nodes * sizeof(yk_bvh_node), hipMemcpyDeviceToHost) != hipSuccess ||
        hipMemcpy(order.data(), d_order.p, (size_t)n_shapes * sizeof(uint32_t), hipMemcpyDeviceToHost) != hipSuccess) {
        (void)hipGetLastError();
        return YK_ERR_DEVICE;
    }
    out.nodes.swap(nodes);
    out.shape_order.swap(order);
    return YK_OK;
}

const HostBvh* scene_host_tree(const yk_scene* s) {
    if (!s || !s->bvh) return nullptr;
    std::lock_guard<std::mutex> lock(s->tree_mu);
    if (s->bvh_lazy && !s->tree_fetched.load() &&
        fetch_tree(s->device, s->tree_nodes, s->tree_order, (uint32_t)s->info.n_nodes, (uint32_t)s->info.n_shapes, *s->bvh_lazy) == YK_OK)
        s->tree_fetched.store(1u);
    return s->tree_fetched.load() ? s->bvh.get() : nullptr;
}

hipError_t upload_host_tree(const HostBvh& bvh, DeviceTree& tree) {
    const std::vector<uint32_t> depth = lay::node_depths(reinterpret_cast<const uint32_t*>(bvh.nodes.data()), bvh.nodes.size());
    tree.n_nodes = (uint32_t)bvh.nodes.size();
    tree.n_shapes = (uint32_t)bvh.shape_order.size();
    std::memcpy(tree.root_words, bvh.nodes.data(), 32);
    hipError_t e = put_host_array(tree.nodes, bvh.nodes.data(), bvh.nodes.size() * sizeof(yk_bvh_node));
    if (e == hipSuccess) e = put_host_array(tree.depth, depth.data(), depth.size() * 4);
    if (e == hipSuccess) e = put_host_array(tree.order, bvh.shape_order.data(), bvh.shape_order.size() * 4);
    return e;
}

void adopt_device_tree(yk_scene* s, DeviceTree& tree, const std::shared_ptr<HostBvh>& lazy) {
    std::swap(s->tree_nodes, tree.nodes);
    std::swap(s->tree_order, tree.order);
    std::swap(s->upd.depth, tree.depth);
    if (lazy) {
        s->bvh_lazy = lazy;
        s->tree_fetched.store(0u);
    }
}

static uint32_t layout_on_device(yk_context* ctx, SceneImage* img, yk_scene* s) {
    const yk_scene_desc* d = img->d;
    DeviceTree& tree = img->dtree;
    double t0 = now_seconds();
    const bool user_order = img->tree_on_device && d->shape_order;
    DevScratch tmp;
    uint8_t* d_mat_kind = nullptr;
    uint32_t* d_user = nullptr;
    if (!tmp.get(d_mat_kind, img->mat_kind.size()) || (user_order && !tmp.get(d_user, tree.n_shapes))) return layout_reason_of(tmp.err);
    hipError_t e = hipMemcpy(d_mat_kind, img->mat_kind.data(), img->mat_kind.size(), hipMemcpyHostToDevice);
    if (e == hipSuccess && user_order) e = hipMemcpy(d_user, d->shape_order, (size_t)tree.n_shapes * 4, hipMemcpyHostToDevice);
    if (e == hipSuccess && !img->tree_on_device) e = upload_host_tree(*img->bvh, tree);
    if (e != hipSuccess) return layout_reason_of(e);
    s->layout.seconds_upload = now_seconds() - t0;
    t0 = now_seconds();
    const uint32_t r = layout_scene_device(ctx, s, tree, d_user, d_mat_kind, d->normals || d->uvs, img->bvh->depth, &img->order_applied);
    s->layout.seconds_layout = now_seconds() - t0;
    if (r != YK_LAYOUT_REASON_NONE) return r;
    if (img->tree_on_device) adopt_device_tree(s, tree, img->bvh_mut);
    tree.release();
    return YK_LAYOUT_REASON_NONE;
}

static yk_status upload_records(yk_context* ctx, yk_scene* s, const SceneRecords& r) {
    yk_status st;
    if ((st = upload(ctx, s->nodes, r.nodes.data(), r.nodes.size())) != YK_OK || (st = upload(ctx, s->nodes4, r.nodes4.data(), r.nodes4.size())) != YK_OK ||
        (st = upload(ctx, s->top_nodes, r.top.data(), r.top.size())) != YK_OK || (st = upload(ctx, s->top_nodes_any, r.top_any.data(), r.top_any.size())) != YK_OK ||
        (st = upload(ctx, s->tris, r.tris.data(), r.tris.size())) != YK_OK || (st = upload(ctx, s->prim_shade, r.prim_shade.data(), r.prim_shade.size())) != YK_OK ||
        (st = upload(ctx, s->prim_attr, r.prim_attr.data(), r.prim_attr.size())) != YK_OK)
        return st;
    set_record_layout(s, s->info.n_interior, r.nodes4.size(), r.top.size(), r.top_any.size(), s->info.n_shapes, !r.prim_attr.empty(), r.root_ref, r.wide_auto);
    return YK_OK;
}

static void bind_records(yk_scene* s) {
    const yk_scene_layout_info& li = s->layout;
    DevScene& ds = s->dev;
    ds.nodes = s->nodes.as<DevNode>();
    ds.nodes4 = li.wide ? s->nodes4.as<DevNode4>() : nullptr;
    s->wide_auto = li.wide_auto != 0;
    ds.top_nodes = s->top_nodes.as<DevNode>();
    ds.n_top = li.n_top;
    ds.top_nodes_any = s->top_nodes_any.as<DevNode>();
    ds.n_top_any = li.n_top_any;
    ds.tris = s->tris.as<float4>();
    ds.prim_shade = s->prim_shade.as<uint4>();
    ds.prim_attr = s->record_bytes[YK_RECORDS_PRIM_ATTR] ? s->prim_attr.as<float4>() : nullptr;
    ds.root_ref = li.root_ref;
    for (int k = 0; k < 3; ++k) {
        ds.root_bmin[k] = s->info.bounds_min[k];
        ds.root_bmax[k] = s->info.bounds_max[k];
    }
}

static void bind_device_scene(yk_scene* s, const yk_scene_desc* d) {
    bind_records(s);
    DevScene& ds = s->dev;
    ds.spheres = d->n_spheres ? s->spheres.as<DevSphere>() : nullptr;
    ds.n_triangles = d->n_triangles;
    for (int k = 0; k < 3; ++k) ds.background[k] = d->background[k];
    ds.indices = s->indices.as<uint32_t>();
    ds.points = s->points.as<float>();
    ds.normals = s->normals.as<float>();
    ds.uvs = s->uvs.as<float>();
    ds.tri_mesh = s->tri_mesh.as<uint32_t>();
    ds.tri_material = s->tri_material.as<int32_t>();
    ds.tri_area_light = s->tri_area_light.as<int32_t>();
    ds.mesh_flags = s->mesh_flags.as<uint32_t>();
    ds.materials = s->materials.as<Material>();
    ds.lights = s->lights.as<DevLight>();
    ds.n_lights = d->n_lights;
    ds.texels = d->n_textures ? s->texels.as<float4>() : nullptr;
    ds.tex_info = d->n_textures ? s->tex_info.as<uint4>() : nullptr;
    s->on_device = true;
    for (DevBuf* b : scene_buffers(s)) s->info.device_bytes += b->bytes;
}

static void init_update_state(yk_scene* s, const yk_scene_desc* d, const LayoutOptions& opt, const std::vector<uint8_t>& mat_kind, bool host_only) {
    yk_scene::UpdateState& u = s->upd;
    u.n_vertices = d->n_vertices;
    u.has_normals = d->normals != nullptr;
    u.has_uvs = d->uvs != nullptr;
    u.opt = opt;
    u.mat_kind = mat_kind;
    u.sphere_bounds.resize(6 * (size_t)d->n_spheres);
    for (uint32_t k = 0; k < d->n_spheres; ++k) {
        const ShapeBounds b = sphere_bound(d->spheres[k]);
        std::memcpy(&u.sphere_bounds[6 * (size_t)k], &b, sizeof(b));
    }
    if (host_only && d->n_triangles) u.host_indices.assign(d->indices, d->indices + 3 * (size_t)d->n_triangles);
}

yk_status yk_upload_scene_image(yk_context* ctx, const std::shared_ptr<SceneImage>& img, yk_scene** out) try {
    if (!out) return fail(ctx, YK_ERR_INVALID_ARGUMENT, "null out");
    *out = nullptr;
    if (!img || !img->bvh) return fail(ctx, YK_ERR_INVALID_ARGUMENT, "null scene image");
    ScenePtr guard(new yk_scene(), yk_scene_destroy);
    yk_scene* s = guard.get();
    s->device = ctx ? ctx->device : -1;
    s->bvh = img->bvh;
    set_scene_counts(s, img->d);
    s->info = img->info;
    s->build_info = img->build_info;
    s->shape_kind = img->shape_kind;
    init_update_state(s, img->d, img->opt, img->mat_kind, ctx == nullptr);
    if (!ctx) {
        const yk_scene_desc* d = img->d;
        SceneImage tables;
        yk_status st = small_tables(nullptr, d, &tables);
        if (st != YK_OK) return st;
        yk_scene::ShadingTables& h = s->host_shading;
        h.mesh_flags.swap(tables.mesh_flags);
        h.materials.swap(tables.mats);
        h.spheres.swap(tables.spheres);
        h.texels.swap(tables.texels);
        h.tex_info.swap(tables.tex_info);
        h.tri_mesh.assign(d->n_triangles, 0);
        if (d->tri_mesh) std::memcpy(h.tri_mesh.data(), d->tri_mesh, sizeof(uint32_t) * d->n_triangles);
        if (d->n_triangles) h.tri_material.assign(d->tri_material, d->tri_material + d->n_triangles);
        if (d->uvs) h.uvs.assign(d->uvs, d->uvs + 2 * (size_t)d->n_vertices);
    }
    if (ctx) {
        if (!img->has_device_records) return fail(ctx, YK_ERR_INVALID_ARGUMENT, "scene image was built without device records");
        const yk_scene_desc* d = img->d;
        (void)hipSetDevice(ctx->device);
        double u0 = now_seconds();
        yk_status st;
#define UP(buf, ptr, n) \
    if ((st = upload(ctx, s->buf, ptr, n)) != YK_OK) return st;
        UP(indices, d->indices, 3 * (size_t)d->n_triangles);
// ... 29 lines not shown
        if (li.layout == YK_LAYOUT_HOST && (st = upload_records(ctx, s, img->rec)) != YK_OK) return st;
        bind_device_scene(s, d);
        s->info.upload_seconds = now_seconds() - u0;
    }
    *out = guard.release();
    return YK_OK;
} YK_CATCH(ctx)

const std::vector<uint8_t>* scene_shape_kind(const yk_scene* s) {
    if (!s) return nullptr;
    if (s->shape_kind_lazy)
        std::call_once(s->kind_once, [s] {
            std::vector<int32_t> mat(s->n_triangles);
            (void)hipSetDevice(s->device);
            if (s->n_triangles && hipMemcpy(mat.data(), s->tri_material.p, (size_t)s->n_triangles * sizeof(int32_t), hipMemcpyDeviceToHost) != hipSuccess) {
                (void)hipGetLastError();
                return;
            }
            std::vector<uint8_t> kinds((size_t)s->n_triangles + s->n_spheres);
            for (uint32_t i = 0; i < s->n_triangles; ++i) kinds[i] = s->lazy_mat_kind[(uint32_t)mat[i]];
            for (uint32_t k = 0; k < s->n_spheres; ++k) kinds[(size_t)s->n_triangles + k] = s->lazy_sphere_kind[k];
            s->shape_kind.swap(kinds);
            s->kind_fetched.store(1u);
        });
    return s->kind_fetched.load() ? &s->shape_kind : nullptr;
}


struct DeviceArray {
    const char* name;
    const void* p;
    size_t bytes;
};
static yk_status check_device_arrays(yk_context* ctx, std::initializer_list<DeviceArray> arrays) {
    for (const DeviceArray& a : arrays) {
        if (!a.p) continue;
        hipPointerAttribute_t at;
        std::memset(&at, 0, sizeof(at));
        const hipError_t e = hipPointerGetAttributes(&at, a.p);
        if (e != hipSuccess) (void)hipGetLastError();
        if (e != hipSuccess || at.type != hipMemoryTypeDevice || at.device != ctx->device) return fail(ctx, YK_ERR_INVALID_ARGUMENT, std::string(a.name) + " is not device memory of this context's device");
        hipDeviceptr_t base = nullptr;
        size_t size = 0;
        if (hipMemGetAddressRange(&base, &size, const_cast<void*>(a.p)) != hipSuccess) {
            (void)hipGetLastError();
        } else if (reinterpret_cast<const char*>(a.p) + a.bytes > reinterpret_cast<const char*>(base) + size) {
            return fail(ctx, YK_ERR_INVALID_ARGUMENT, std::string(a.name) + " is shorter than its count says");
        }
    }
    return YK_OK;
}

static yk_status create_scene_on_device(yk_context* ctx, const yk_scene_desc* d, hipStream_t st, yk_scene** out, bool* fall_back, yk_bvh_build_info* refused) {
    *fall_back = false;
    std::memset(refused, 0, sizeof(*refused));
    const uint32_t nt = d->n_triangles, N = nt + d->n_spheres;
    ScenePtr guard(new yk_scene(), yk_scene_destroy);
    yk_scene* s = guard.get();
    s->device = ctx->device;
    set_scene_counts(s, d);
    std::memset(&s->info, 0, sizeof(s->info));
    std::memset(&s->build_info, 0, sizeof(s->build_info));
    const double u0 = now_seconds();

    auto own = [&](DevBuf& buf, const void* src, size_t bytes, int fill) -> hipError_t {
        hipError_t e = buf.ensure(std::max<size_t>(bytes, 16));
        if (e != hipSuccess || bytes == 0) return e;
        return src ? hipMemcpyAsync(buf.p, src, bytes, hipMemcpyDeviceToDevice, st) : hipMemsetAsync(buf.p, fill, bytes, st);
    };
    HIP_TRY(ctx, own(s->indices, d->indices, 12 * (size_t)nt, 0));
    HIP_TRY(ctx, own(s->points, d->points, 12 * (size_t)d->n_vertices, 0));
    HIP_TRY(ctx, own(s->normals, d->normals, d->normals ? 12 * (size_t)d->n_vertices : 0, 0));
    HIP_TRY(ctx, own(s->uvs, d->uvs, d->uvs ? 8 * (size_t)d->n_vertices : 0, 0));
    HIP_TRY(ctx, own(s->tri_mesh, d->tri_mesh, 4 * (size_t)nt, 0));
    HIP_TRY(ctx, own(s->tri_material, d->tri_material, 4 * (size_t)nt, 0));
    HIP_TRY(ctx, own(s->tri_area_light, d->tri_area_light, 4 * (size_t)nt, 0xff));

    SceneImage img;
    std::memset(&img.info, 0, sizeof(img.info));
    yk_status rc = small_tables(ctx, d, &img);
    if (rc != YK_OK) return rc;
    std::vector<uint8_t> light_kind(std::max<uint32_t>(d->n_lights, 1), 0);
    std::vector<uint8_t>& mat_kind = img.mat_kind;
    init_update_state(s, d, LayoutOptions{ctx->top_nodes, ctx->wide_bvh}, mat_kind, false);
    for (uint32_t l = 0; l < d->n_lights; ++l) light_kind[l] = (uint8_t)d->lights[l].kind;
    std::vector<ShapeBounds> sphere_b(std::max<uint32_t>(d->n_spheres, 1));
    for (uint32_t k = 0; k < d->n_spheres; ++k) sphere_b[k] = sphere_bound(d->spheres[k]);

    DevScratch tmp;
    inp::CheckWords* d_words = nullptr;
    uint8_t *d_light_kind = nullptr, *d_mat_kind = nullptr;
    uint32_t *d_seen = nullptr, *d_user = nullptr;
    float *d_sphere_b = nullptr, *d_sb = nullptr;
    if (!tmp.get(d_words, 1) || !tmp.get(d_light_kind, light_kind.size()) || !tmp.get(d_mat_kind, mat_kind.size()) || !tmp.get(d_sphere_b, 6 * sphere_b.size()) || !tmp.get(d_sb, 6 * (size_t)N) ||
        (d->shape_order && (!tmp.get(d_seen, ((size_t)N + 31) / 32) || !tmp.get(d_user, N))))
        return fail(ctx, YK_ERR_OUT_OF_MEMORY, "no device memory for the scene's input stage");
    HIP_TRY(ctx, hipMemcpyAsync(d_light_kind, light_kind.data(), light_kind.size(), hipMemcpyHostToDevice, st));
    HIP_TRY(ctx, hipMemcpyAsync(d_mat_kind, mat_kind.data(), mat_kind.size(), hipMemcpyHostToDevice, st));
    HIP_TRY(ctx, hipMemcpyAsync(d_sphere_b, sphere_b.data(), sphere_b.size() * sizeof(ShapeBounds), hipMemcpyHostToDevice, st));
    if (d->shape_order) HIP_TRY(ctx, hipMemcpyAsync(d_user, d->shape_order, 4 * (size_t)N, hipMemcpyDeviceToDevice, st));

    inp::Geometry g;
    g.indices = s->indices.as<uint32_t>();
    g.tri_mesh = d->tri_mesh ? s->tri_mesh.as<uint32_t>() : nullptr;
    g.tri_material = s->tri_material.as<int32_t>();
    g.tri_area_light = d->tri_area_light ? s->tri_area_light.as<int32_t>() : nullptr;
    g.n_triangles = nt;
    g.n_vertices = d->n_vertices;
    g.n_meshes = d->n_meshes;
    g.n_materials = d->n_materials;
    g.n_lights = d->n_lights;
    inp::CheckWords words;
    HIP_TRY(ctx, enqueue_geometry_checks(st, g, d_light_kind, d_user, N, d_seen, d_words));
    HIP_TRY(ctx, hipMemcpyAsync(&words, d_words, sizeof(words), hipMemcpyDeviceToHost, st));
    HIP_TRY(ctx, hipStreamSynchronize(st));
    if (words.first != inp::kNoFailure) {
        static const char* const what[4] = {"vertex index out of range", "mesh index out of range", "material index out of range", "light index out of range"};
        return fail(ctx, YK_ERR_INVALID_ARGUMENT, what[words.first & 3u]);
    }
    if (words.light != inp::kNoFailure) return fail(ctx, YK_ERR_INVALID_ARGUMENT, "tri_area_light must be -1 or index a rectangular light");
    if (words.order_bad) return fail(ctx, YK_ERR_INVALID_ARGUMENT, "shape_order is not a permutation of the shapes");

    const double t0 = now_seconds();
    HIP_TRY(ctx, enqueue_shape_bounds(st, s->points.as<float>(), s->indices.as<uint32_t>(), d_user, d_sphere_b, nt, N, d_sb, d_words));
    HIP_TRY(ctx, hipMemcpyAsync(&words.non_finite, &d_words->non_finite, sizeof(uint32_t), hipMemcpyDeviceToHost, st));
    HIP_TRY(ctx, hipStreamSynchronize(st));
    if (words.non_finite) {
        refused->small_range = (uint32_t)ctx->bvh_small_range;
        refused->reason = YK_BVH_REASON_NON_FINITE;
        *fall_back = true;
        return YK_OK;
    }
    img.bvh = img.bvh_mut = std::make_shared<HostBvh>();
    img.tree_on_device = true;
    if (!build_bvh_device(ctx, nullptr, d_sb, N, d->max_shapes_in_node, d->split_method, (uint32_t)ctx->bvh_small_range, *img.bvh_mut, s->build_info, &img.dtree)) {
        *refused = s->build_info;
        *fall_back = true;
        return YK_OK;
    }
    img.info.build_seconds = now_seconds() - t0;
    if (img.bvh->split_failed || img.dtree.n_nodes == 0) return fail(ctx, YK_ERR_BVH_BUILD, "BVH split failed (reference: assert_ne!(mid, start))");
    fill_scene_info(&img);
    if (img.info.n_nodes > YK_REF_INDEX_MAX || img.info.n_shapes > YK_REF_INDEX_MAX) return fail(ctx, YK_ERR_UNSUPPORTED, "more than 2^28 BVH nodes or shapes");
    s->info = img.info;

    if ((rc = upload(ctx, s->mesh_flags, img.mesh_flags.data(), img.mesh_flags.size())) != YK_OK || (rc = upload(ctx, s->materials, img.mats.data(), img.mats.size())) != YK_OK ||
        (rc = upload(ctx, s->lights, img.lights.data(), img.lights.size())) != YK_OK || (rc = upload(ctx, s->spheres, img.spheres.data(), img.spheres.size())) != YK_OK ||
        (rc = upload(ctx, s->texels, img.texels.data(), img.texels.size())) != YK_OK || (rc = upload(ctx, s->tex_info, img.tex_info.data(), img.tex_info.size())) != YK_OK)
        return rc;
    const double l0 = now_seconds();
    bool order_applied = false;
    if (layout_scene_device(ctx, s, img.dtree, d_user, d_mat_kind, d->normals || d->uvs, img.bvh->depth, &order_applied) != YK_LAYOUT_REASON_NONE) {
        *fall_back = true;
        return YK_OK;
    }
    s->layout.layout = YK_LAYOUT_DEVICE;
    s->layout.seconds_layout = now_seconds() - l0;
    s->bvh = img.bvh;
    adopt_device_tree(s, img.dtree, img.bvh_mut);
    s->lazy_mat_kind.swap(mat_kind);
    s->lazy_sphere_kind.resize(d->n_spheres);
    for (uint32_t k = 0; k < d->n_spheres; ++k) s->lazy_sphere_kind[k] = s->lazy_mat_kind[(uint32_t)d->spheres[k].material];
    s->shape_kind_lazy = true;
    s->kind_fetched.store(0u);
    bind_device_scene(s, d);
    s->info.upload_seconds = now_seconds() - u0;
    *out = guard.release();
// ... 222 lines not shown
    if (ctx) {
        (void)hipSetDevice(ctx->device);
        if ((rc = drain_context(ctx)) != YK_OK) return rc;
    }
    if (ctx && s->layout.layout == YK_LAYOUT_DEVICE) {
        DevScratch tmp;
        float *d_points = nullptr, *d_normals = nullptr;
        if (tmp.get(d_points, n) && (!normals || tmp.get(d_normals, n)) && hipMemcpy(d_points, points, n * 4, hipMemcpyHostToDevice) == hipSuccess &&
            (!normals || hipMemcpy(d_normals, normals, n * 4, hipMemcpyHostToDevice) == hipSuccess)) {
            rc = update_scene(ctx, s, d_points, d_normals, points, normals);
        } else {
            (void)hipGetLastError();
            rc = update_scene_host(ctx, s, points, normals, YK_LAYOUT_REASON_OUT_OF_MEMORY);
        }
    } else {
        rc = update_scene_host(ctx, s, points, normals, YK_LAYOUT_REASON_NONE);
    }
    if (rc == YK_OK) finish_update(s, t_begin);
    return rc;
} YK_CATCH(ctx)

yk_status yk_scene_update_device(yk_context* ctx, yk_scene* s, const float* d_points, const float* d_normals, void* stream) try {
    if (!ctx) return YK_ERR_INVALID_ARGUMENT;
    YK_LOCK(ctx);
    const double t_begin = now_seconds();
    yk_status rc = check_update(ctx, s, d_points, d_normals);
    if (rc != YK_OK) return rc;
    (void)hipSetDevice(ctx->device);
    const size_t bytes = 12 * (size_t)s->upd.n_vertices;
    if ((rc = check_device_arrays(ctx, {{"points", d_points, bytes}, {"normals", d_normals, bytes}})) != YK_OK) return rc;
    if (stream) {
        HIP_TRY(ctx, hipEventRecord(ctx->ev_in, (hipStream_t)stream));
        HIP_TRY(ctx, hipStreamWaitEvent(ctx->stream, ctx->ev_in, 0));
    }
    if ((rc = drain_context(ctx)) != YK_OK) return rc;
    rc = update_scene(ctx, s, d_points, d_normals, nullptr, nullptr);
    if (rc == YK_OK) finish_update(s, t_begin);
    return rc;
} YK_CATCH(ctx)

yk_status yk_scene_get_update_info(const yk_scene* s, yk_scene_update_info* out) {
    if (!s || !out) return YK_ERR_INVALID_ARGUMENT;
    *out = s->upd.info;
    return YK_OK;
}

void yk_scene_destroy(yk_scene* s) {
    if (!s) return;
    if (s->device >= 0) (void)hipSetDevice(s->device);
    for (DevBuf* b : scene_buffers(s)) b->release();
    for (DevBuf* b : {&s->upd.depth, &s->upd.list, &s->upd.sphere_b, &s->upd.mat_kind_d, &s->upd.words}) b->release();
    delete s;
}

yk_status yk_scene_get_info(const yk_scene* s, yk_scene_info* out) {
    if (!s || !out) return YK_ERR_INVALID_ARGUMENT;
    *out = s->info;
    return YK_OK;
}

yk_status yk_scene_get_build_info(const yk_scene* s, yk_bvh_build_info* out) {
    if (!s || !out) return YK_ERR_INVALID_ARGUMENT;
    *out = s->build_info;
    return YK_OK;
}

yk_status yk_scene_export_bvh(const yk_scene* s, yk_bvh_node* nodes, uint32_t* shape_order) {
    if (!s) return YK_ERR_INVALID_ARGUMENT;
    const HostBvh* bvh = scene_host_tree(s);
    if (!bvh) return YK_ERR_DEVICE;
    if (nodes) std::memcpy(nodes, bvh->nodes.data(), bvh->nodes.size() * sizeof(yk_bvh_node));
    if (shape_order) std::memcpy(shape_order, bvh->shape_order.data(), bvh->shape_order.size() * sizeof(uint32_t));
    return YK_OK;
}

yk_status yk_scene_get_layout_info(const yk_scene* s, yk_scene_layout_info* out) {
    if (!s || !out) return YK_ERR_INVALID_ARGUMENT;
    *out = s->layout;
    out->tree_fetched = s->tree_fetched.load();
    return YK_OK;
}

yk_status yk_scene_read_records(const yk_scene* s, uint32_t which, void* out, size_t cap_bytes, size_t* n_bytes) {
    if (!s || !s->on_device || which > YK_RECORDS_PRIM_ATTR || !n_bytes) return YK_ERR_INVALID_ARGUMENT;
    const DevBuf& buf = record_buffer(s, which);
    const size_t bytes = s->record_bytes[which];
    *n_bytes = bytes;
    if (!out) return YK_OK;
    if (cap_bytes < bytes || buf.bytes < bytes) return YK_ERR_INVALID_ARGUMENT;
    (void)hipSetDevice(s->device);
    if (bytes && hipMemcpy(out, buf.p, bytes, hipMemcpyDeviceToHost) != hipSuccess) {
        (void)hipGetLastError();
        return YK_ERR_DEVICE;
    }
    return YK_OK;
}

}
```

### yuki_amd/csrc/yk_scene_layout.h

```cpp
#pragma once
#include <stddef.h>
#include <stdint.h>

#include <vector>

#include "yk_bvh_build.h"
#include "yk_device.h"

namespace yk {
namespace lay {

using lv::kNone;

YK_HD bool nd_leaf(const uint32_t* nodes, uint32_t i) { return (nodes[8 * (size_t)i + 7] >> 24) != 0u; }
YK_HD uint32_t nd_a(const uint32_t* nodes, uint32_t i) { return nodes[8 * (size_t)i + 6]; }
YK_HD uint32_t nd_count(const uint32_t* nodes, uint32_t i) { return nodes[8 * (size_t)i + 7] & 0xffffu; }
YK_HD uint32_t nd_axis(const uint32_t* nodes, uint32_t i) { return (nodes[8 * (size_t)i + 7] >> 16) & 0xffu; }

inline std::vector<uint32_t> node_depths(const uint32_t* nodes, size_t n) {
    std::vector<uint32_t> depth(n, 0u);
    depth[0] = 1u;
    for (uint32_t i = 0; i < (uint32_t)n; ++i)
        if (!nd_leaf(nodes, i)) depth[i + 1u] = depth[nd_a(nodes, i)] = depth[i] + 1u;
    return depth;
// ... 37 lines not shown
        uint32_t total;
        const uint32_t t0 = size + ex.scan((i0 ? 1u : 0u) + (i1 ? 1u : 0u), total), t1 = t0 + (i0 ? 1u : 0u);
        const bool a0 = i0 && t0 < cap, a1 = i1 && t1 < cap;
        if (a0) order[t0] = c0;
        if (a1) order[t1] = c1;
        if (in && id0) {
            id0[q] = a0 ? t0 : kNone;
            id1[q] = a1 ? t1 : kNone;
        }
        size = size + total < cap ? size + total : cap;
        done = end;
        ex.sync();
    }
    return size;
}

YK_HD bool wide_collapsed(const uint32_t* nodes, const uint32_t* depth, uint32_t i) { return !nd_leaf(nodes, i) && ((depth[i] ^ depth[0]) & 1u) == 0u; }
YK_HD void wide_children(const uint32_t* nodes, uint32_t P, uint32_t (&child)[4]) {
    const uint32_t A = P + 1u, B = nd_a(nodes, P);
    const bool la = nd_leaf(nodes, A), lb = nd_leaf(nodes, B);
    child[0] = la ? A : A + 1u;
    child[1] = la ? YK_REF_NONE : nd_a(nodes, A);
    child[2] = lb ? B : B + 1u;
    child[3] = lb ? YK_REF_NONE : nd_a(nodes, B);
}
YK_HD uint32_t wide_count(const uint32_t* nodes, const uint32_t* depth, uint32_t i) {
    if (!wide_collapsed(nodes, depth, i)) return 0u;
    uint32_t child[4], n = 0u;
    wide_children(nodes, i, child);
#pragma unroll
    for (int k = 0; k < 4; ++k) n += (child[k] != YK_REF_NONE && !nd_leaf(nodes, child[k])) ? 1u : 0u;
    return n;
}
YK_HD void wide_refs(const uint32_t* nodes, uint32_t excl, const uint32_t (&child)[4], uint32_t (&ref)[4], uint32_t* slot_of) {
    uint32_t next = 1u + excl;
#pragma unroll
    for (int k = 0; k < 4; ++k) {
        if (child[k] == YK_REF_NONE) {
            ref[k] = YK_REF_NONE;
        } else if (nd_leaf(nodes, child[k])) {
            ref[k] = YK_LEAF_BIT | nd_a(nodes, child[k]);
        } else {
            ref[k] = next;
            if (slot_of) slot_of[child[k]] = next;
            ++next;
        }
    }
}
YK_HD void dev_node4_words(const uint32_t* nodes, uint32_t P, const uint32_t (&child)[4], const uint32_t (&ref)[4], uint4 (&q)[8]) {
    const uint4 zero = make_uint4(0u, 0u, 0u, 0u);
    NodeWords c[4];
#pragma unroll
    for (int k = 0; k < 4; ++k) {
        c[k].lo = zero;
        c[k].hi = zero;
        if (child[k] != YK_REF_NONE) c[k] = load_node(nodes, child[k]);
    }
#pragma unroll
    for (int h = 0; h < 2; ++h) {
        const NodeWords &u = c[2 * h], &v = c[2 * h + 1];
        q[3 * h + 0] = u.lo;
        q[3 * h + 1] = make_uint4(u.hi.x, u.hi.y, v.lo.x, v.lo.y);
        q[3 * h + 2] = make_uint4(v.lo.z, v.lo.w, v.hi.x, v.hi.y);
    }
    const uint32_t A = P + 1u, B = nd_a(nodes, P);
    const uint32_t axA = nd_leaf(nodes, A) ? 0u : nd_axis(nodes, A), axB = nd_leaf(nodes, B) ? 0u : nd_axis(nodes, B);
    q[6] = make_uint4(ref[0], ref[1], ref[2], ref[3]);
    q[7] = make_uint4(nd_axis(nodes, P) | (axA << 2) | (axB << 4), 0u, 0u, 0u);
}

struct PrimArrays {
    const uint32_t* indices;
    const float* points;
    const float* normals;
    const float* uvs;
    const uint32_t* tri_mesh;
    const int32_t* tri_material;
    const int32_t* tri_area_light;
    const uint32_t* mesh_flags;
    const DevSphere* spheres;
    const uint8_t* mat_kind;
    uint32_t n_triangles;
};
YK_HD void prim_words(const PrimArrays& s, uint32_t src, bool last, uint4 (&tri)[3], uint4& shade, uint4 (&attr)[4], bool want_attr) {
    const uint4 zero = make_uint4(0u, 0u, 0u, 0u);
#pragma unroll
    for (int k = 0; k < 4; ++k) attr[k] = zero;
    if (src >= s.n_triangles) {
        const uint32_t mat = (uint32_t)s.spheres[src - s.n_triangles].material, kind = s.mat_kind[mat];
        tri[0] = make_uint4(0u, 0u, 0u, 0xffffffffu);
        tri[1] = make_uint4(0u, 0u, 0u, src);
        tri[2] = make_uint4(0u, 0u, 0u, (last ? YK_PRIM_LAST : 0u) | YK_PRIM_SPHERE | (kind << YK_PRIM_KIND_SHIFT));
        shade = make_uint4(0u, 0u, 0u, (mat << 6) | (kind << 3));
        return;
    }
    const uint32_t vi[3] = {s.indices[3 * (size_t)src], s.indices[3 * (size_t)src + 1], s.indices[3 * (size_t)src + 2]};
    const uint32_t mat = (uint32_t)s.tri_material[src], kind = s.mat_kind[mat], mfl = s.mesh_flags[s.tri_mesh[src]];
    const uint32_t w[3] = {(uint32_t)s.tri_area_light[src], src, (last ? YK_PRIM_LAST : 0u) | (kind << YK_PRIM_KIND_SHIFT)};
#pragma unroll
    for (int k = 0; k < 3; ++k) {
        const float* p = s.points + 3 * (size_t)vi[k];
        tri[k] = make_uint4(lv::f2u(p[0]), lv::f2u(p[1]), lv::f2u(p[2]), w[k]);
    }
    shade = make_uint4(vi[0], vi[1], vi[2], (mat << 6) | (kind << 3) | mfl);
    if (!want_attr) return;
    uint32_t nrm[3][3] = {}, uv[3][2] = {};
#pragma unroll
    for (int k = 0; k < 3; ++k) {
        if (mfl & YK_MESH_NORMALS)
            for (int c = 0; c < 3; ++c) nrm[k][c] = lv::f2u(s.normals[3 * (size_t)vi[k] + c]);
        if (mfl & YK_MESH_UVS)
            for (int c = 0; c < 2; ++c) uv[k][c] = lv::f2u(s.uvs[2 * (size_t)vi[k] + c]);
    }
    attr[0] = make_uint4(nrm[0][0], nrm[0][1], nrm[0][2], uv[0][0]);
    attr[1] = make_uint4(nrm[1][0], nrm[1][1], nrm[1][2], uv[0][1]);
    attr[2] = make_uint4(nrm[2][0], nrm[2][1], nrm[2][2], uv[1][0]);
    attr[3] = make_uint4(uv[1][1], uv[2][0], uv[2][1], 0u);
}

}
}
```

### yuki_amd/csrc/yk_scene_layout.hip

```cpp
#include <hip/hip_runtime.h>

#include <algorithm>
#include <cstring>
#include <vector>

#include "yk_internal.h"
#include "yk_scan.h"
#include "yk_scene_layout.h"

using namespace yk::lay;
using namespace yk::scan;

namespace {

const int kThreads = 256;

struct HostExec {
    uint32_t tid = 0, nt = 1;
    void sync() {}
    uint32_t scan(uint32_t v, uint32_t& total) {
        total = v;
        return 0u;
    }
};
struct WaveExec {
    uint32_t tid, nt;
    __device__ void sync() { __syncthreads(); }
    __device__ uint32_t scan(uint32_t v, uint32_t& total) {
        const uint32_t inc = wave_incl_scan(v, tid);
        total = __shfl(inc, 63);
        return inc - v;
    }
};

struct IsInterior {
    const uint32_t* __restrict__ nodes;
    __device__ uint32_t operator()(uint32_t i) const { return nd_leaf(nodes, i) ? 0u : 1u; }
};
struct WideCount {
    const uint32_t *__restrict__ nodes, *__restrict__ depth;
    __device__ uint32_t operator()(uint32_t i) const { return wide_count(nodes, depth, i); }
};

__global__ void k_apply_order(uint32_t* order, const uint32_t* __restrict__ user, uint32_t np) {
    const uint32_t p = blockIdx.x * blockDim.x + threadIdx.x;
    if (p < np) order[p] = user[order[p]];
}
__global__ void k_nodes(const uint32_t* __restrict__ nodes, const uint32_t* __restrict__ iidx, uint32_t n, uint4* out, uint8_t* last) {
    const uint32_t i = blockIdx.x * blockDim.x + threadIdx.x;
    if (i >= n) return;
    if (nd_leaf(nodes, i)) {
        last[(size_t)nd_a(nodes, i) + nd_count(nodes, i) - 1u] = 1;
        return;
    }
    uint4 q[4];
    dev_node_words(nodes, i, ref_of(nodes, iidx, i + 1u), ref_of(nodes, iidx, nd_a(nodes, i)), q);
    uint4* o = out + 4 * (size_t)iidx[i];
#pragma unroll
    for (int k = 0; k < 4; ++k) o[k] = q[k];
}
__global__ void __launch_bounds__(64) k_tops(const uint32_t* __restrict__ nodes, const uint32_t* __restrict__ iidx, uint32_t cap_closest, uint32_t cap_any, uint4* out_closest, uint4* out_any, uint32_t* words) {
    __shared__ uint32_t order[YK_TOP_MAX], id0[YK_TOP_MAX], id1[YK_TOP_MAX];
    const uint32_t cap = blockIdx.x == 0 ? cap_closest : cap_any;
    uint4* out = blockIdx.x == 0 ? out_closest : out_any;
    WaveExec ex{threadIdx.x, blockDim.x};
    const uint32_t size = top_order(ex, nodes, cap, order, id0, id1);
    for (uint32_t q = threadIdx.x; q < size; q += blockDim.x) {
        const uint32_t P = order[q];
        const uint32_t r0 = id0[q] != kNone ? (YK_TOP_BIT | id0[q]) : ref_of(nodes, iidx, P + 1u);
        const uint32_t r1 = id1[q] != kNone ? (YK_TOP_BIT | id1[q]) : ref_of(nodes, iidx, nd_a(nodes, P));
        uint4 w[4];
        dev_node_words(nodes, P, r0, r1, w);
        uint4* o = out + 4 * (size_t)q;
#pragma unroll
        for (int k = 0; k < 4; ++k) o[k] = w[k];
    }
    if (threadIdx.x == 0) words[2 + blockIdx.x] = size;
}
__global__ void k_wide_slots(const uint32_t* __restrict__ nodes, const uint32_t* __restrict__ depth, const uint32_t* __restrict__ excl, uint32_t n, uint32_t* slot) {
    const uint32_t i = blockIdx.x * blockDim.x + threadIdx.x;
    if (i >= n || !wide_collapsed(nodes, depth, i)) return;
    if (i == 0u) slot[0] = 0u;
    uint32_t child[4], ref[4];
    wide_children(nodes, i, child);
    wide_refs(nodes, excl[i], child, ref, slot);
}
__global__ void k_wide_nodes(const uint32_t* __restrict__ nodes, const uint32_t* __restrict__ depth, const uint32_t* __restrict__ excl, const uint32_t* __restrict__ slot, uint32_t n, uint32_t n4, uint4* out) {
    const uint32_t i = blockIdx.x * blockDim.x + threadIdx.x;
    if (i >= n || !wide_collapsed(nodes, depth, i)) return;
    const uint32_t me = slot[i];
    if (me >= n4) return;
    uint32_t child[4], ref[4];
    wide_children(nodes, i, child);
    wide_refs(nodes, excl[i], child, ref, nullptr);
    uint4 q[8];
    dev_node4_words(nodes, i, child, ref, q);
    uint4* o = out + 8 * (size_t)me;
#pragma unroll
    for (int k = 0; k < 8; ++k) o[k] = q[k];
}
__global__ void k_prims(PrimArrays s, const uint32_t* __restrict__ order, const uint8_t* __restrict__ last, uint32_t np, uint32_t n_shapes_total, uint4* tris, uint4* prim_shade, uint4* prim_attr) {
    const uint32_t p = blockIdx.x * blockDim.x + threadIdx.x;
    if (p >= np) return;
    const uint32_t src = order[p];
    if (src >= n_shapes_total) return;
    uint4 tri[3], shade, attr[4];
    prim_words(s, src, last[p] != 0, tri, shade, attr, prim_attr != nullptr);
#pragma unroll
    for (int k = 0; k < 3; ++k) tris[3 * (size_t)p + k] = tri[k];
    prim_shade[p] = shade;
    if (prim_attr) {
#pragma unroll
        for (int k = 0; k < 4; ++k) prim_attr[4 * (size_t)p + k] = attr[k];
    }
}

unsigned blocks(size_t n, int threads) { return (unsigned)((n + threads - 1) / threads); }

}

uint32_t layout_scene_device(yk_context* ctx, yk_scene* s, const DeviceTree& tree, const uint32_t* d_user_order, const uint8_t* d_mat_kind, bool has_attr, uint32_t tree_depth, bool* order_applied) {
    const uint32_t n = tree.n_nodes, np = tree.n_shapes;
    if (n == 0 || np == 0 || n > YK_REF_INDEX_MAX || np > YK_REF_INDEX_MAX) return YK_LAYOUT_REASON_DEVICE_ERROR;
    (void)hipSetDevice(ctx->device);
    hipStream_t st = ctx->stream;
    const uint32_t* nodes = tree.nodes.as<uint32_t>();
    const uint32_t* depth = tree.depth.as<uint32_t>();
    uint32_t* order = tree.order.as<uint32_t>();
    const bool root_leaf = (tree.root_words[7] >> 24) != 0u;
    const uint32_t n_interior = (n - 1u) / 2u;
    const uint32_t cap_closest = (uint32_t)std::min<int64_t>(std::min<int64_t>(s->upd.opt.top_nodes, trace_top_nodes()), YK_TOP_MAX);
    const uint32_t cap_any = (uint32_t)std::min<int64_t>(std::min<int64_t>(s->upd.opt.top_nodes, trace_top_nodes_any()), YK_TOP_MAX);
    const bool wide = s->upd.opt.wide_bvh != 0 && !root_leaf && tree_depth <= 64;

    DevScratch tmp;
    uint32_t *d_index = nullptr, *d_bsum = nullptr, *d_slot = nullptr, *d_words = nullptr;
    uint8_t* d_last = nullptr;
    if (!tmp.get(d_index, n) || !tmp.get(d_bsum, scan_blocks(n)) || !tmp.get(d_last, np) || !tmp.get(d_words, 16) || (wide && !tmp.get(d_slot, n))) return YK_LAYOUT_REASON_OUT_OF_MEMORY;
#define LAY_TRY(expr)                                                                                   \
    do {                                                                                                \
        const hipError_t e_ = (expr);                                                                   \
        if (e_ != hipSuccess) {                                                                         \
            (void)hipStreamSynchronize(st);                                                             \
            return layout_reason_of(e_);                                                                \
        }                                                                                               \
    } while (0)
    LAY_TRY(s->nodes.ensure(std::max<size_t>(n_interior, 1) * sizeof(DevNode)));
    LAY_TRY(s->top_nodes.ensure(std::max<size_t>((size_t)std::min(cap_closest, n_interior) * sizeof(DevNode), 16)));
    LAY_TRY(s->top_nodes_any.ensure(std::max<size_t>((size_t)std::min(cap_any, n_interior) * sizeof(DevNode), 16)));
    LAY_TRY(s->tris.ensure(3 * (size_t)np * sizeof(float4)));
    LAY_TRY(s->prim_shade.ensure((size_t)np * sizeof(uint4)));
    LAY_TRY(s->prim_attr.ensure(has_attr ? 4 * (size_t)np * sizeof(float4) : 16));

    LAY_TRY(hipMemsetAsync(d_words, 0, 16 * sizeof(uint32_t), st));
    LAY_TRY(hipMemsetAsync(d_last, 0, np, st));
    if (d_user_order) {
        k_apply_order<<<blocks(np, kThreads), kThreads, 0, st>>>(order, d_user_order, np);
        LAY_TRY(hipGetLastError());
        *order_applied = true;
    }
    enqueue_scan(st, IsInterior{nodes}, n, d_index, d_bsum, d_words + 0, true);
    if (n_interior == 0) LAY_TRY(hipMemsetAsync(s->nodes.p, 0, sizeof(DevNode), st));
    k_nodes<<<blocks(n, kThreads), kThreads, 0, st>>>(nodes, d_index, n, s->nodes.as<uint4>(), d_last);
    k_tops<<<2, 64, 0, st>>>(nodes, d_index, std::min(cap_closest, n_interior), std::min(cap_any, n_interior), s->top_nodes.as<uint4>(), s->top_nodes_any.as<uint4>(), d_words);
    LAY_TRY(hipGetLastError());
    PrimArrays pa;
    pa.indices = s->indices.as<uint32_t>();
    pa.points = s->points.as<float>();
    pa.normals = s->normals.as<float>();
    pa.uvs = s->uvs.as<float>();
    pa.tri_mesh = s->tri_mesh.as<uint32_t>();
    pa.tri_material = s->tri_material.as<int32_t>();
    pa.tri_area_light = s->tri_area_light.as<int32_t>();
    pa.mesh_flags = s->mesh_flags.as<uint32_t>();
    pa.spheres = s->spheres.as<DevSphere>();
    pa.mat_kind = d_mat_kind;
    pa.n_triangles = s->n_triangles;
    k_prims<<<blocks(np, kThreads), kThreads, 0, st>>>(pa, order, d_last, np, s->n_triangles + s->n_spheres, s->tris.as<uint4>(), s->prim_shade.as<uint4>(), has_attr ? s->prim_attr.as<uint4>() : nullptr);
    LAY_TRY(hipGetLastError());
    uint32_t words[16];
    if (wide) {
        enqueue_scan(st, WideCount{nodes, depth}, n, d_index, d_bsum, d_words + 1, true);
        k_wide_slots<<<blocks(n, kThreads), kThreads, 0, st>>>(nodes, depth, d_index, n, d_slot);
        LAY_TRY(hipGetLastError());
    }
    LAY_TRY(hipMemcpyAsync(words, d_words, sizeof(words), hipMemcpyDeviceToHost, st));
    LAY_TRY(hipStreamSynchronize(st));
    if (words[0] != n_interior) return YK_LAYOUT_REASON_DEVICE_ERROR;
    uint32_t n4 = 0;
    if (wide) {
        n4 = 1u + words[1];
        if (n4 > n_interior) return YK_LAYOUT_REASON_DEVICE_ERROR;
        LAY_TRY(s->nodes4.ensure((size_t)n4 * sizeof(DevNode4)));
        k_wide_nodes<<<blocks(n, kThreads), kThreads, 0, st>>>(nodes, depth, d_index, d_slot, n, n4, s->nodes4.as<uint4>());
        LAY_TRY(hipGetLastError());
        LAY_TRY(hipStreamSynchronize(st));
    } else {
        LAY_TRY(s->nodes4.ensure(16));
    }
#undef LAY_TRY
    set_record_layout(s, n_interior, n4, words[2], words[3], np, has_attr, root_leaf ? (YK_LEAF_BIT | tree.root_words[6]) : 0u, wide && s->upd.opt.wide_bvh == 2);
    return YK_LAYOUT_REASON_NONE;
}

extern "C" size_t yk_layout_top_order(const yk_bvh_node* nodes, size_t n, uint32_t cap, uint32_t* out_order) try {
    if (!nodes || n == 0 || n > YK_REF_INDEX_MAX || (cap && !out_order)) return 0;
    const uint32_t* w = reinterpret_cast<const uint32_t*>(nodes);
    HostExec ex;
    return top_order(ex, w, cap, out_order, (uint32_t*)nullptr, (uint32_t*)nullptr);
} catch (const std::exception&) {
    return 0;
}

extern "C" size_t yk_layout_wide_slots(const yk_bvh_node* nodes, size_t n, uint32_t* out_slot_per_node) try {
    if (!nodes || n == 0 || n > YK_REF_INDEX_MAX || !out_slot_per_node) return 0;
    const uint32_t* w = reinterpret_cast<const uint32_t*>(nodes);
    for (size_t i = 0; i < n; ++i) out_slot_per_node[i] = kNone;
    if (nd_leaf(w, 0u)) return 0;
    const std::vector<uint32_t> depth = node_depths(w, n);
    std::vector<uint32_t> excl(n);
    uint32_t run = 0u;
    for (uint32_t i = 0; i < (uint32_t)n; ++i) {
        excl[i] = run;
        run += wide_count(w, depth.data(), i);
    }
    out_slot_per_node[0] = 0u;
    for (uint32_t i = 0; i < (uint32_t)n; ++i) {
        if (!wide_collapsed(w, depth.data(), i)) continue;
        uint32_t child[4], ref[4];
        wide_children(w, i, child);
        wide_refs(w, excl[i], child, ref, out_slot_per_node);
    }
    return 1u + (size_t)run;
} catch (const std::exception&) {
    return 0;
}
```

### yuki_amd/csrc/yk_scene_records.cpp

```cpp
#include "yk_scene_records.h"

#include <algorithm>
#include <cstring>

#include "yk_kernels.h"

using namespace yk;

static void layout_nodes(const HostLayoutInput& in, SceneRecords& out) {
    const std::vector<yk_bvh_node>& nodes = in.bvh->nodes;
    std::vector<uint32_t> interior_index(nodes.size());
    uint32_t cnt = 0;
    for (size_t i = 0; i < nodes.size(); ++i) {
        interior_index[i] = cnt;
        if (!nodes[i].is_leaf) ++cnt;
    }
    auto ref_of = [&](uint32_t idx) -> uint32_t { return nodes[idx].is_leaf ? (YK_LEAF_BIT | nodes[idx].a) : interior_index[idx]; };
    std::vector<DevNode>& dn = out.nodes;
    dn.assign(std::max<size_t>(in.n_interior, 1), DevNode());
    for (size_t i = 0; i < nodes.size(); ++i) {
        if (nodes[i].is_leaf) continue;
        const yk_bvh_node& c0 = nodes[i + 1];
        const yk_bvh_node& c1 = nodes[nodes[i].a];
        DevNode& o = dn[interior_index[i]];
        o.q0 = make_float4(c0.bmin[0], c0.bmin[1], c0.bmin[2], c0.bmax[0]);
        o.q1 = make_float4(c0.bmax[1], c0.bmax[2], c1.bmin[0], c1.bmin[1]);
        o.q2 = make_float4(c1.bmin[2], c1.bmax[0], c1.bmax[1], c1.bmax[2]);
        o.q3 = make_uint4(ref_of((uint32_t)i + 1), ref_of(nodes[i].a) | ((uint32_t)nodes[i].axis << YK_AXIS_SHIFT), 0u, 0u);
    }
    auto build_top = [&](size_t cap, std::vector<DevNode>& top) {
        top.clear();
        if (nodes[0].is_leaf || cap == 0) return;
        std::vector<uint32_t> order;
        std::vector<uint32_t> top_id(nodes.size(), 0xffffffffu);
        order.push_back(0);
        top_id[0] = 0;
        for (size_t q = 0; q < order.size() && order.size() < cap; ++q) {
            const uint32_t P = order[q];
            for (uint32_t c : {P + 1, nodes[P].a}) {
                if (!nodes[c].is_leaf && order.size() < cap) {
                    top_id[c] = (uint32_t)order.size();
                    order.push_back(c);
                }
            }
        }
        for (uint32_t P : order) {
            DevNode t = dn[interior_index[P]];
            const uint32_t c0 = P + 1, c1 = nodes[P].a;
            if (top_id[c0] != 0xffffffffu) t.q3.x = YK_TOP_BIT | top_id[c0];
            if (top_id[c1] != 0xffffffffu) t.q3.y = YK_TOP_BIT | top_id[c1] | ((uint32_t)nodes[P].axis << YK_AXIS_SHIFT);
            top.push_back(t);
        }
    };
    build_top((size_t)std::min<int64_t>(in.opt.top_nodes, trace_top_nodes()), out.top);
    build_top((size_t)std::min<int64_t>(in.opt.top_nodes, trace_top_nodes_any()), out.top_any);
    out.root_ref = ref_of(0);
}

static void layout_wide(const HostLayoutInput& in, SceneRecords& out) {
    const std::vector<yk_bvh_node>& nodes = in.bvh->nodes;
    std::vector<DevNode4>& dn4 = out.nodes4;
    const bool wide = in.opt.wide_bvh != 0 && !nodes[0].is_leaf && in.bvh->depth <= 64;
    out.wide_auto = wide && in.opt.wide_bvh == 2;
    if (!wide) return;
    dn4.reserve(in.n_interior / 2 + 1);
    struct Todo {
        uint32_t binary;
        uint32_t slot;
    };
    std::vector<Todo> stack;
    dn4.emplace_back();
    stack.push_back(Todo{0u, 0u});
    while (!stack.empty()) {
        const Todo td = stack.back();
        stack.pop_back();
        const uint32_t P = td.binary, A = P + 1, B = nodes[P].a;
        uint32_t child[4] = {YK_REF_NONE, YK_REF_NONE, YK_REF_NONE, YK_REF_NONE};
        if (nodes[A].is_leaf) {
            child[0] = A;
        } else {
            child[0] = A + 1;
            child[1] = nodes[A].a;
        }
        if (nodes[B].is_leaf) {
            child[2] = B;
        } else {
            child[2] = B + 1;
            child[3] = nodes[B].a;
// ... 5 lines not shown
            if (child[k] == YK_REF_NONE) continue;
            const yk_bvh_node& c = nodes[child[k]];
            for (int a = 0; a < 3; ++a) {
                box[k][a] = c.bmin[a];
                box[k][3 + a] = c.bmax[a];
            }
            if (c.is_leaf) {
                ref[k] = YK_LEAF_BIT | c.a;
            } else {
                ref[k] = (uint32_t)dn4.size();
                dn4.emplace_back();
            }
        }
        for (int k = 3; k >= 0; --k)
            if (ref[k] != YK_REF_NONE && !(ref[k] & YK_LEAF_BIT)) stack.push_back(Todo{child[k], ref[k]});
        DevNode4& o = dn4[td.slot];
        o.q0 = make_float4(box[0][0], box[0][1], box[0][2], box[0][3]);
        o.q1 = make_float4(box[0][4], box[0][5], box[1][0], box[1][1]);
        o.q2 = make_float4(box[1][2], box[1][3], box[1][4], box[1][5]);
        o.q3 = make_float4(box[2][0], box[2][1], box[2][2], box[2][3]);
        o.q4 = make_float4(box[2][4], box[2][5], box[3][0], box[3][1]);
        o.q5 = make_float4(box[3][2], box[3][3], box[3][4], box[3][5]);
        o.q6 = make_uint4(ref[0], ref[1], ref[2], ref[3]);
        const uint32_t axA = nodes[A].is_leaf ? 0u : nodes[A].axis, axB = nodes[B].is_leaf ? 0u : nodes[B].axis;
        o.q7 = make_uint4((uint32_t)nodes[P].axis | (axA << 2) | (axB << 4), 0u, 0u, 0u);
    }
}

static void layout_prims(const HostLayoutInput& in, SceneRecords& out) {
    const HostBvh* bvh = in.bvh;
    const uint32_t nt = in.n_triangles;
    const size_t np = bvh->shape_order.size();
    auto bits = [](uint32_t u) {
        float f;
        std::memcpy(&f, &u, 4);
        return f;
    };
    out.tris.assign(3 * np, make_float4(0.0f, 0.0f, 0.0f, 0.0f));
    out.prim_shade.assign(np, make_uint4(0u, 0u, 0u, 0u));
    std::vector<uint8_t> last(np, 0);
    for (const yk_bvh_node& n : bvh->nodes)
        if (n.is_leaf) last[(size_t)n.a + n.count - 1] = 1;
    for (size_t p = 0; p < np; ++p) {
        const uint32_t src = bvh->shape_order[p];
        const uint32_t material = (uint32_t)(src >= nt ? in.sphere_material[src - nt] : in.tri_material[src]), kind = in.mat_kind[material];
        const uint32_t flags = (last[p] ? YK_PRIM_LAST : 0u) | (kind << YK_PRIM_KIND_SHIFT);
        if (src >= nt) {
            out.tris[3 * p + 0] = make_float4(0.0f, 0.0f, 0.0f, bits(0xffffffffu));
            out.tris[3 * p + 1] = make_float4(0.0f, 0.0f, 0.0f, bits(src));
            out.tris[3 * p + 2] = make_float4(0.0f, 0.0f, 0.0f, bits(flags | YK_PRIM_SPHERE));
            out.prim_shade[p] = make_uint4(0u, 0u, 0u, (material << 6) | (kind << 3));
            continue;
        }
        const uint32_t* vi = in.indices + 3 * (size_t)src;
        const float* p0 = in.points + 3 * (size_t)vi[0];
        const float* p1 = in.points + 3 * (size_t)vi[1];
        const float* p2 = in.points + 3 * (size_t)vi[2];
        out.tris[3 * p + 0] = make_float4(p0[0], p0[1], p0[2], bits((uint32_t)in.tri_area_light[src]));
        out.tris[3 * p + 1] = make_float4(p1[0], p1[1], p1[2], bits(src));
        out.tris[3 * p + 2] = make_float4(p2[0], p2[1], p2[2], bits(flags));
        out.prim_shade[p] = make_uint4(vi[0], vi[1], vi[2], (material << 6) | (kind << 3) | in.mesh_flags[in.tri_mesh[src]]);
    }
    if (!in.normals && !in.uvs) return;
    out.prim_attr.assign(4 * np, make_float4(0.0f, 0.0f, 0.0f, 0.0f));
    for (size_t p = 0; p < np; ++p) {
        const uint32_t src = bvh->shape_order[p];
        if (src >= nt) continue;
        const uint32_t mfl = in.mesh_flags[in.tri_mesh[src]];
        float nrm[3][3] = {}, uv[3][2] = {};
        for (int k = 0; k < 3; ++k) {
            const size_t vi = in.indices[3 * (size_t)src + k];
            if (mfl & YK_MESH_NORMALS)
                for (int c = 0; c < 3; ++c) nrm[k][c] = in.normals[3 * vi + c];
            if (mfl & YK_MESH_UVS)
                for (int c = 0; c < 2; ++c) uv[k][c] = in.uvs[2 * vi + c];
        }
        out.prim_attr[4 * p + 0] = make_float4(nrm[0][0], nrm[0][1], nrm[0][2], uv[0][0]);
        out.prim_attr[4 * p + 1] = make_float4(nrm[1][0], nrm[1][1], nrm[1][2], uv[0][1]);
        out.prim_attr[4 * p + 2] = make_float4(nrm[2][0], nrm[2][1], nrm[2][2], uv[1][0]);
        out.prim_attr[4 * p + 3] = make_float4(uv[1][1], uv[2][0], uv[2][1], 0.0f);
    }
}

SceneRecords layout_records_host(const HostLayoutInput& in) {
    SceneRecords out;
    layout_nodes(in, out);
    layout_wide(in, out);
    layout_prims(in, out);
    return out;
}
```

### yuki_amd/csrc/yk_scene_records.h

```cpp
#pragma once
#include <cstdint>
#include <vector>

#include "yk_device.h"
#include "yk_host.h"

struct LayoutOptions {
    int64_t top_nodes = 0, wide_bvh = 0;
};

struct HostLayoutInput {
    const yk::HostBvh* bvh = nullptr;
    uint64_t n_interior = 0;
    const uint32_t* indices = nullptr;
    const float *points = nullptr, *normals = nullptr, *uvs = nullptr;
    const int32_t *tri_material = nullptr, *tri_area_light = nullptr;
    const uint32_t *tri_mesh = nullptr, *mesh_flags = nullptr;
    uint32_t n_triangles = 0;
    const int32_t* sphere_material = nullptr;
    const uint8_t* mat_kind = nullptr;
    LayoutOptions opt;
};

struct SceneRecords {
    std::vector<yk::DevNode> nodes;
    std::vector<yk::DevNode4> nodes4;
    std::vector<yk::DevNode> top, top_any;
    std::vector<float4> tris;
    std::vector<uint4> prim_shade;
    std::vector<float4> prim_attr;
    uint32_t root_ref = 0;
    bool wide_auto = false;
};

SceneRecords layout_records_host(const HostLayoutInput& in);
```

Before: 2292 Mray/s.

## Pack per-primitive shading data into one 128-byte fused record

```diff
diff --git a/include/yuki_hip.h b/include/yuki_hip.h
--- a/include/yuki_hip.h
+++ b/include/yuki_hip.h
@@ -242,8 +242,9 @@
     uint32_t root_ref, n_top, n_top_any, wide, wide_auto;
 } yk_scene_layout_info;
 yk_status yk_scene_get_layout_info(const yk_scene* scene, yk_scene_layout_info* out);
-enum { YK_RECORDS_NODES = 0, YK_RECORDS_NODES4 = 1, YK_RECORDS_TOP = 2, YK_RECORDS_TOP_ANY = 3, YK_RECORDS_TRIS = 4, YK_RECORDS_PRIM_SHADE = 5, YK_RECORDS_PRIM_ATTR = 6 };
+enum { YK_RECORDS_NODES = 0, YK_RECORDS_NODES4 = 1, YK_RECORDS_TOP = 2, YK_RECORDS_TOP_ANY = 3, YK_RECORDS_TRIS = 4, YK_RECORDS_PRIM_SHADE = 5, YK_RECORDS_PRIM_ATTR = 6, YK_RECORDS_PRIM_REC = 7 };
 yk_status yk_scene_read_records(const yk_scene* scene, uint32_t which, void* out, size_t cap_bytes, size_t* n_bytes);
+yk_status yk_layout_records_host(const yk_scene_desc* desc, uint32_t which, void* out, size_t cap_bytes, size_t* n_bytes);
 size_t yk_layout_top_order(const yk_bvh_node* nodes, size_t n, uint32_t cap, uint32_t* out_order);
 size_t yk_layout_wide_slots(const yk_bvh_node* nodes, size_t n, uint32_t* out_slot_per_node);
 size_t yk_bvh_partition_plan(const uint8_t* pass, size_t n, uint32_t* order);
diff --git a/yuki_amd/_ffi.py b/yuki_amd/_ffi.py
--- a/yuki_amd/_ffi.py
+++ b/yuki_amd/_ffi.py
@@ -112,6 +112,7 @@
     "yk_bvh_partition_plan": (C.c_size_t, [vp, C.c_size_t, vp]),
     "yk_scene_get_layout_info": (C.c_int, [vp, C.POINTER(abi.SceneLayoutInfo)]),
     "yk_scene_read_records": (C.c_int, [vp, C.c_uint32, vp, C.c_size_t, C.POINTER(C.c_size_t)]),
+    "yk_layout_records_host": (C.c_int, [C.POINTER(abi.SceneDesc), C.c_uint32, vp, C.c_size_t, C.POINTER(C.c_size_t)]),
     "yk_layout_top_order": (C.c_size_t, [vp, C.c_size_t, C.c_uint32, vp]),
     "yk_layout_wide_slots": (C.c_size_t, [vp, C.c_size_t, vp]),
     "yk_render_tiles": (C.c_int, [vp, vp, C.POINTER(abi.CameraMatrices), C.POINTER(abi.SamplerDesc), C.POINTER(abi.IntegratorDesc), vp, C.c_size_t, vp, C.POINTER(RenderStats), vp, vp]),
diff --git a/yuki_amd/abi.py b/yuki_amd/abi.py
--- a/yuki_amd/abi.py
+++ b/yuki_amd/abi.py
@@ -262,8 +262,8 @@
 LAYOUT_HOST, LAYOUT_DEVICE = 0, 1
 UPDATE_ROUTE_HOST, UPDATE_ROUTE_DEVICE = 0, 1
 LAYOUT_REASON_NONE, LAYOUT_REASON_OUT_OF_MEMORY, LAYOUT_REASON_DEVICE_ERROR, LAYOUT_REASON_MULTI = 0, 1, 2, 3
-RECORDS_NODES, RECORDS_NODES4, RECORDS_TOP, RECORDS_TOP_ANY, RECORDS_TRIS, RECORDS_PRIM_SHADE, RECORDS_PRIM_ATTR = range(7)
-RECORD_NAMES = ("nodes", "nodes4", "top", "top_any", "tris", "prim_shade", "prim_attr")
+RECORDS_NODES, RECORDS_NODES4, RECORDS_TOP, RECORDS_TOP_ANY, RECORDS_TRIS, RECORDS_PRIM_SHADE, RECORDS_PRIM_ATTR, RECORDS_PRIM_REC = range(8)
+RECORD_NAMES = ("nodes", "nodes4", "top", "top_any", "tris", "prim_shade", "prim_attr", "prim_rec")
 
 
 def ptr(a, ty):
diff --git a/yuki_amd/core.py b/yuki_amd/core.py
--- a/yuki_amd/core.py
+++ b/yuki_amd/core.py
@@ -1002,6 +1002,18 @@
     return address, stream
 
 
+def host_layout_records(scene_data, which):
+    if isinstance(which, str):
+        which = abi.RECORD_NAMES.index(which)
+    d, keep = scene_data.desc(LightFactory)
+    n = C.c_size_t(0)
+    check(lib().yk_layout_records_host(C.byref(d), int(which), None, 0, C.byref(n)))
+    out = np.zeros(n.value, dtype=np.uint8)
+    check(lib().yk_layout_records_host(C.byref(d), int(which), _p(out), out.nbytes, C.byref(n)))
+    del keep
+    return out
+
+
 class Scene:
 
     def __init__(self, ctx, scene_data):
diff --git a/yuki_amd/csrc/yk_context.cpp b/yuki_amd/csrc/yk_context.cpp
--- a/yuki_amd/csrc/yk_context.cpp
+++ b/yuki_amd/csrc/yk_context.cpp
@@ -181,6 +181,9 @@
     } else if (k == "scene_layout") {
         if (value < 0 || value > 1) return YK_ERR_INVALID_ARGUMENT;
         ctx->scene_layout = value;
+    } else if (k == "shade_records") {
+        if (value < 0 || value > 1) return YK_ERR_INVALID_ARGUMENT;
+        ctx->shade_records = value;
     } else if (k == "trace_stage_kernel") {
         if (value < 0 || value > 2) return YK_ERR_INVALID_ARGUMENT;
         ctx->trace_stage_kernel = value;
diff --git a/yuki_amd/csrc/yk_device.h b/yuki_amd/csrc/yk_device.h
--- a/yuki_amd/csrc/yk_device.h
+++ b/yuki_amd/csrc/yk_device.h
@@ -60,6 +60,13 @@
 #define YK_MESH_UVS 2u
 #define YK_MESH_SWAPS 4u
 
+struct DevPrimRec {
+    float4 q0, q1, q2;
+    uint4 q3;
+    float4 q4, q5, q6, q7;
+};
+static_assert(sizeof(DevPrimRec) == 128 && sizeof(DevPrimRec[2]) == 256, "DevPrimRec: one 128-byte line a slot");
+
 struct DevScene {
     const DevNode* nodes;
     const DevNode4* nodes4;
@@ -70,6 +77,7 @@
     const float4* tris;
     const uint4* prim_shade;
     const float4* prim_attr;
+    const DevPrimRec* prim_rec;
     const DevSphere* spheres;
     uint32_t n_triangles;
     uint32_t root_ref;
diff --git a/yuki_amd/csrc/yk_geom.h b/yuki_amd/csrc/yk_geom.h
--- a/yuki_amd/csrc/yk_geom.h
+++ b/yuki_amd/csrc/yk_geom.h
@@ -261,8 +261,22 @@
 }
 
 YK_HD Surface hit_surface_prim(const DevScene& sc, uint32_t prim, V3 o, V3 d, bool want_uv, float* t_out, uint4* id_out) {
-    const float4 v0 = sc.tris[3 * prim], v1 = sc.tris[3 * prim + 1], v2 = sc.tris[3 * prim + 2];
-    const uint4 ps = sc.prim_shade[prim];
+    const bool fused = sc.prim_rec != nullptr;
+    float4 v0, v1, v2;
+    uint4 ps;
+    if (fused) {
+        const DevPrimRec& r = sc.prim_rec[prim];
+        v0 = r.q0;
+        v1 = r.q1;
+        v2 = r.q2;
+        const uint4 q3 = r.q3;
+        ps = make_uint4(q3.y, q3.z, q3.w, q3.x);
+    } else {
+        v0 = sc.tris[3 * prim];
+        v1 = sc.tris[3 * prim + 1];
+        v2 = sc.tris[3 * prim + 2];
+        ps = sc.prim_shade[prim];
+    }
     const uint32_t src = __float_as_uint(v1.w);
     if (__float_as_uint(v2.w) & YK_PRIM_SPHERE) {
         const DevSphere& sp = sc.spheres[src - sc.n_triangles];
@@ -276,8 +290,9 @@
     TriAttr at;
     at.u0x = at.u0y = at.u1x = at.u1y = at.u2x = at.u2y = 0.0f;
     at.n0 = at.n1 = at.n2 = V3{0.0f, 0.0f, 0.0f};
-    if (sc.prim_attr && (ps.w & (YK_MESH_NORMALS | YK_MESH_UVS))) {
-        const float4 a0 = sc.prim_attr[4 * (size_t)prim], a1 = sc.prim_attr[4 * (size_t)prim + 1], a2 = sc.prim_attr[4 * (size_t)prim + 2], a3 = sc.prim_attr[4 * (size_t)prim + 3];
+    if ((fused || sc.prim_attr) && (ps.w & (YK_MESH_NORMALS | YK_MESH_UVS))) {
+        const float4* a = fused ? reinterpret_cast<const float4*>(sc.prim_rec + prim) + 4 : sc.prim_attr + 4 * (size_t)prim;
+        const float4 a0 = a[0], a1 = a[1], a2 = a[2], a3 = a[3];
         at.n0 = V3{a0.x, a0.y, a0.z};
         at.n1 = V3{a1.x, a1.y, a1.z};
         at.n2 = V3{a2.x, a2.y, a2.z};
@@ -291,7 +306,7 @@
     tri_intersect(o, rt, __builtin_inff(), p0, p1, p2, th);
     if (t_out) *t_out = th.t;
     if (id_out) *id_out = make_uint4(src, __float_as_uint(th.b0), __float_as_uint(th.b1), __float_as_uint(th.b2));
-    Surface s = sc.prim_attr ? make_surface_vals(p0, p1, p2, at, ps.w & 7u, th) : make_surface_core(sc, p0, p1, p2, ps.x, ps.y, ps.z, ps.w & 7u, th);
+    Surface s = (fused || sc.prim_attr) ? make_surface_vals(p0, p1, p2, at, ps.w & 7u, th) : make_surface_core(sc, p0, p1, p2, ps.x, ps.y, ps.z, ps.w & 7u, th);
     s.material = (int)(ps.w >> 6);
     s.area_light = (int)__float_as_uint(v0.w);
     s.wo = -d;
diff --git a/yuki_amd/csrc/yk_internal.h b/yuki_amd/csrc/yk_internal.h
--- a/yuki_amd/csrc/yk_internal.h
+++ b/yuki_amd/csrc/yk_internal.h
@@ -88,6 +88,7 @@
     int64_t top_nodes = YK_TOP_MAX;
     int64_t bvh_builder = 0;
     int64_t bvh_small_range = YK_BVH_SMALL_RANGE;
+    int64_t shade_records = 1;
     int64_t scene_layout = 0;
     int64_t trace_stage_kernel = 0;
     int64_t update_top_block = 1;
@@ -171,7 +172,7 @@
     mutable std::mutex tree_mu;
     mutable std::atomic<uint32_t> tree_fetched{1};
     yk_scene_layout_info layout = {};
-    size_t record_bytes[7] = {};
+    size_t record_bytes[8] = {};
     uint32_t n_triangles = 0, n_spheres = 0, n_lights = 0, n_delta_lights = 0;
     uint32_t n_materials = 0, n_meshes = 0, n_textures = 0;
     bool wide_auto = false;
@@ -182,7 +183,7 @@
     bool shape_kind_lazy = false;
     mutable std::once_flag kind_once;
     mutable std::atomic<uint32_t> kind_fetched{1};
-    DevBuf nodes, nodes4, top_nodes, top_nodes_any, tris, prim_shade, prim_attr, indices, points, normals, uvs, tri_mesh, tri_material, tri_area_light, mesh_flags, materials, lights, spheres, texels, tex_info;
+    DevBuf nodes, nodes4, top_nodes, top_nodes_any, tris, prim_shade, prim_attr, prim_rec, indices, points, normals, uvs, tri_mesh, tri_material, tri_area_light, mesh_flags, materials, lights, spheres, texels, tex_info;
     DevScene dev;
     bool on_device = false;
     struct UpdateState {
@@ -299,7 +300,7 @@
 
 yk_status adaptive_select_into(yk_context* ctx, hipStream_t st, const yk_adaptive_desc* desc, const void* d_stats, yk_pixel_list* list, uint32_t* out_n);
 
-void set_record_layout(yk_scene* s, size_t n_interior, size_t n_wide, size_t n_top, size_t n_top_any, size_t n_shapes, bool has_attr, uint32_t root_ref, bool wide_auto);
+void set_record_layout(yk_scene* s, size_t n_interior, size_t n_wide, size_t n_top, size_t n_top_any, size_t n_shapes, bool has_attr, bool has_rec, uint32_t root_ref, bool wide_auto);
 hipError_t upload_host_tree(const HostBvh& bvh, DeviceTree& tree);
 void adopt_device_tree(yk_scene* s, DeviceTree& tree, const std::shared_ptr<HostBvh>& lazy);
 Material make_material(const yk_material_desc& m);
diff --git a/yuki_amd/csrc/yk_scene.cpp b/yuki_amd/csrc/yk_scene.cpp
--- a/yuki_amd/csrc/yk_scene.cpp
+++ b/yuki_amd/csrc/yk_scene.cpp
@@ -97,13 +97,13 @@
     return d;
 }
 
-static std::array<DevBuf*, 22> scene_buffers(yk_scene* s) {
-    return {&s->nodes,    &s->nodes4,       &s->top_nodes,      &s->top_nodes_any, &s->tris,      &s->prim_shade, &s->prim_attr, &s->indices, &s->points,  &s->normals,    &s->uvs,
+static std::array<DevBuf*, 23> scene_buffers(yk_scene* s) {
+    return {&s->nodes,    &s->nodes4,       &s->top_nodes,      &s->top_nodes_any, &s->tris,      &s->prim_shade, &s->prim_attr, &s->prim_rec, &s->indices, &s->points,  &s->normals,    &s->uvs,
             &s->tri_mesh, &s->tri_material, &s->tri_area_light, &s->mesh_flags,    &s->materials, &s->lights,     &s->spheres,   &s->texels,  &s->tex_info, &s->tree_nodes, &s->tree_order};
 }
 static const DevBuf& record_buffer(const yk_scene* s, uint32_t which) { return *scene_buffers(const_cast<yk_scene*>(s))[which]; }
 
-void set_record_layout(yk_scene* s, size_t n_interior, size_t n_wide, size_t n_top, size_t n_top_any, size_t n_shapes, bool has_attr, uint32_t root_ref, bool wide_auto) {
+void set_record_layout(yk_scene* s, size_t n_interior, size_t n_wide, size_t n_top, size_t n_top_any, size_t n_shapes, bool has_attr, bool has_rec, uint32_t root_ref, bool wide_auto) {
     yk_scene_layout_info& li = s->layout;
     li.root_ref = root_ref;
     li.n_top = (uint32_t)n_top;
@@ -117,6 +117,7 @@
     s->record_bytes[YK_RECORDS_TRIS] = 3 * n_shapes * sizeof(float4);
     s->record_bytes[YK_RECORDS_PRIM_SHADE] = n_shapes * sizeof(uint4);
     s->record_bytes[YK_RECORDS_PRIM_ATTR] = has_attr ? 4 * n_shapes * sizeof(float4) : 0;
+    s->record_bytes[YK_RECORDS_PRIM_REC] = has_rec ? n_shapes * sizeof(DevPrimRec) : 0;
 }
 
 struct SceneImage {
@@ -342,7 +343,7 @@
     s->d = d;
     s->device_layout = ctx && what.device_layout;
     s->layout_reason = ctx ? what.layout_reason : 0u;
-    if (ctx) s->opt = LayoutOptions{ctx->top_nodes, ctx->wide_bvh};
+    if (ctx) s->opt = LayoutOptions{ctx->top_nodes, ctx->wide_bvh, ctx->shade_records};
     std::memset(&s->info, 0, sizeof(s->info));
 
     std::vector<ShapeBounds> sb;
@@ -431,9 +432,9 @@
     if ((st = upload(ctx, s->nodes, r.nodes.data(), r.nodes.size())) != YK_OK || (st = upload(ctx, s->nodes4, r.nodes4.data(), r.nodes4.size())) != YK_OK ||
         (st = upload(ctx, s->top_nodes, r.top.data(), r.top.size())) != YK_OK || (st = upload(ctx, s->top_nodes_any, r.top_any.data(), r.top_any.size())) != YK_OK ||
         (st = upload(ctx, s->tris, r.tris.data(), r.tris.size())) != YK_OK || (st = upload(ctx, s->prim_shade, r.prim_shade.data(), r.prim_shade.size())) != YK_OK ||
-        (st = upload(ctx, s->prim_attr, r.prim_attr.data(), r.prim_attr.size())) != YK_OK)
+        (st = upload(ctx, s->prim_attr, r.prim_attr.data(), r.prim_attr.size())) != YK_OK || (st = upload(ctx, s->prim_rec, r.prim_rec.data(), r.prim_rec.size())) != YK_OK)
         return st;
-    set_record_layout(s, s->info.n_interior, r.nodes4.size(), r.top.size(), r.top_any.size(), s->info.n_shapes, !r.prim_attr.empty(), r.root_ref, r.wide_auto);
+    set_record_layout(s, s->info.n_interior, r.nodes4.size(), r.top.size(), r.top_any.size(), s->info.n_shapes, !r.prim_attr.empty(), !r.prim_rec.empty(), r.root_ref, r.wide_auto);
     return YK_OK;
 }
 
@@ -450,6 +451,7 @@
     ds.tris = s->tris.as<float4>();
     ds.prim_shade = s->prim_shade.as<uint4>();
     ds.prim_attr = s->record_bytes[YK_RECORDS_PRIM_ATTR] ? s->prim_attr.as<float4>() : nullptr;
+    ds.prim_rec = s->record_bytes[YK_RECORDS_PRIM_REC] ? s->prim_rec.as<DevPrimRec>() : nullptr;
     ds.root_ref = li.root_ref;
     for (int k = 0; k < 3; ++k) {
         ds.root_bmin[k] = s->info.bounds_min[k];
@@ -645,7 +647,7 @@
     if (rc != YK_OK) return rc;
     std::vector<uint8_t> light_kind(std::max<uint32_t>(d->n_lights, 1), 0);
     std::vector<uint8_t>& mat_kind = img.mat_kind;
-    init_update_state(s, d, LayoutOptions{ctx->top_nodes, ctx->wide_bvh}, mat_kind, false);
+    init_update_state(s, d, LayoutOptions{ctx->top_nodes, ctx->wide_bvh, ctx->shade_records}, mat_kind, false);
     for (uint32_t l = 0; l < d->n_lights; ++l) light_kind[l] = (uint8_t)d->lights[l].kind;
     std::vector<ShapeBounds> sphere_b(std::max<uint32_t>(d->n_spheres, 1));
     for (uint32_t k = 0; k < d->n_spheres; ++k) sphere_b[k] = sphere_bound(d->spheres[k]);
@@ -1034,7 +1036,7 @@
 }
 
 yk_status yk_scene_read_records(const yk_scene* s, uint32_t which, void* out, size_t cap_bytes, size_t* n_bytes) {
-    if (!s || !s->on_device || which > YK_RECORDS_PRIM_ATTR || !n_bytes) return YK_ERR_INVALID_ARGUMENT;
+    if (!s || !s->on_device || which > YK_RECORDS_PRIM_REC || !n_bytes) return YK_ERR_INVALID_ARGUMENT;
     const DevBuf& buf = record_buffer(s, which);
     const size_t bytes = s->record_bytes[which];
     *n_bytes = bytes;
@@ -1048,4 +1050,24 @@
     return YK_OK;
 }
 
-}
+yk_status yk_layout_records_host(const yk_scene_desc* d, uint32_t which, void* out, size_t cap_bytes, size_t* n_bytes) try {
+    if (!d || which > YK_RECORDS_PRIM_REC || !n_bytes) return YK_ERR_INVALID_ARGUMENT;
+    std::shared_ptr<SceneImage> img;
+    yk_status st = yk_build_scene_image(nullptr, d, img, SceneBuild{false, false, 0u});
+    if (st != YK_OK || (st = host_tables(nullptr, d, img.get())) != YK_OK) return st;
+    img->opt = LayoutOptions{YK_TOP_MAX, 2, 1};
+    layout_image_host(img.get());
+    const SceneRecords& r = img->rec;
+    const void* const data[8] = {r.nodes.data(), r.nodes4.data(), r.top.data(), r.top_any.data(), r.tris.data(), r.prim_shade.data(), r.prim_attr.data(), r.prim_rec.data()};
+    const size_t bytes[8] = {r.nodes.size() * sizeof(DevNode),  r.nodes4.size() * sizeof(DevNode4),    r.top.size() * sizeof(DevNode),       r.top_any.size() * sizeof(DevNode),
+                             r.tris.size() * sizeof(float4),    r.prim_shade.size() * sizeof(uint4),   r.prim_attr.size() * sizeof(float4),  r.prim_rec.size() * sizeof(DevPrimRec)};
+    *n_bytes = bytes[which];
+    if (!out) return YK_OK;
+    if (cap_bytes < bytes[which]) return YK_ERR_INVALID_ARGUMENT;
+    if (bytes[which]) std::memcpy(out, data[which], bytes[which]);
+    return YK_OK;
+} catch (const std::exception&) {
+    return YK_ERR_INVALID_ARGUMENT;
+}
+
+}
diff --git a/yuki_amd/csrc/yk_scene_layout.h b/yuki_amd/csrc/yk_scene_layout.h
--- a/yuki_amd/csrc/yk_scene_layout.h
+++ b/yuki_amd/csrc/yk_scene_layout.h
@@ -143,7 +143,15 @@
     const uint8_t* mat_kind;
     uint32_t n_triangles;
 };
-YK_HD void prim_words(const PrimArrays& s, uint32_t src, bool last, uint4 (&tri)[3], uint4& shade, uint4 (&attr)[4], bool want_attr) {
+YK_HD void prim_rec_words(const uint4 (&tri)[3], const uint4& shade, const uint4 (&attr)[4], uint4 (&rec)[8]) {
+    rec[0] = tri[0];
+    rec[1] = tri[1];
+    rec[2] = tri[2];
+    rec[3] = make_uint4(shade.w, shade.x, shade.y, shade.z);
+#pragma unroll
+    for (int k = 0; k < 4; ++k) rec[4 + k] = attr[k];
+}
+YK_HD void prim_words(const PrimArrays& s, uint32_t src, bool last, uint4 (&tri)[3], uint4& shade, uint4 (&attr)[4], bool want_attr, uint4 (*rec)[8]) {
     const uint4 zero = make_uint4(0u, 0u, 0u, 0u);
 #pragma unroll
     for (int k = 0; k < 4; ++k) attr[k] = zero;
@@ -153,6 +161,7 @@
         tri[1] = make_uint4(0u, 0u, 0u, src);
         tri[2] = make_uint4(0u, 0u, 0u, (last ? YK_PRIM_LAST : 0u) | YK_PRIM_SPHERE | (kind << YK_PRIM_KIND_SHIFT));
         shade = make_uint4(0u, 0u, 0u, (mat << 6) | (kind << 3));
+        if (rec) prim_rec_words(tri, shade, attr, *rec);
         return;
     }
     const uint32_t vi[3] = {s.indices[3 * (size_t)src], s.indices[3 * (size_t)src + 1], s.indices[3 * (size_t)src + 2]};
@@ -164,7 +173,10 @@
         tri[k] = make_uint4(lv::f2u(p[0]), lv::f2u(p[1]), lv::f2u(p[2]), w[k]);
     }
     shade = make_uint4(vi[0], vi[1], vi[2], (mat << 6) | (kind << 3) | mfl);
-    if (!want_attr) return;
+    if (!want_attr) {
+        if (rec) prim_rec_words(tri, shade, attr, *rec);
+        return;
+    }
     uint32_t nrm[3][3] = {}, uv[3][2] = {};
 #pragma unroll
     for (int k = 0; k < 3; ++k) {
@@ -177,6 +189,7 @@
     attr[1] = make_uint4(nrm[1][0], nrm[1][1], nrm[1][2], uv[0][1]);
     attr[2] = make_uint4(nrm[2][0], nrm[2][1], nrm[2][2], uv[1][0]);
     attr[3] = make_uint4(uv[1][1], uv[2][0], uv[2][1], 0u);
+    if (rec) prim_rec_words(tri, shade, attr, *rec);
 }
 
 }
diff --git a/yuki_amd/csrc/yk_scene_layout.hip b/yuki_amd/csrc/yk_scene_layout.hip
--- a/yuki_amd/csrc/yk_scene_layout.hip
+++ b/yuki_amd/csrc/yk_scene_layout.hip
@@ -99,19 +99,23 @@
 #pragma unroll
     for (int k = 0; k < 8; ++k) o[k] = q[k];
 }
-__global__ void k_prims(PrimArrays s, const uint32_t* __restrict__ order, const uint8_t* __restrict__ last, uint32_t np, uint32_t n_shapes_total, uint4* tris, uint4* prim_shade, uint4* prim_attr) {
+__global__ void k_prims(PrimArrays s, const uint32_t* __restrict__ order, const uint8_t* __restrict__ last, uint32_t np, uint32_t n_shapes_total, uint4* tris, uint4* prim_shade, uint4* prim_attr, uint4* prim_rec) {
     const uint32_t p = blockIdx.x * blockDim.x + threadIdx.x;
     if (p >= np) return;
     const uint32_t src = order[p];
     if (src >= n_shapes_total) return;
-    uint4 tri[3], shade, attr[4];
-    prim_words(s, src, last[p] != 0, tri, shade, attr, prim_attr != nullptr);
+    uint4 tri[3], shade, attr[4], rec[8];
+    prim_words(s, src, last[p] != 0, tri, shade, attr, prim_attr != nullptr, prim_rec ? &rec : nullptr);
 #pragma unroll
     for (int k = 0; k < 3; ++k) tris[3 * (size_t)p + k] = tri[k];
     prim_shade[p] = shade;
     if (prim_attr) {
 #pragma unroll
         for (int k = 0; k < 4; ++k) prim_attr[4 * (size_t)p + k] = attr[k];
+    }
+    if (prim_rec) {
+#pragma unroll
+        for (int k = 0; k < 8; ++k) prim_rec[8 * (size_t)p + k] = rec[k];
     }
 }
 
@@ -151,6 +155,8 @@
     LAY_TRY(s->tris.ensure(3 * (size_t)np * sizeof(float4)));
     LAY_TRY(s->prim_shade.ensure((size_t)np * sizeof(uint4)));
     LAY_TRY(s->prim_attr.ensure(has_attr ? 4 * (size_t)np * sizeof(float4) : 16));
+    const bool has_rec = s->upd.opt.shade_records != 0;
+    LAY_TRY(s->prim_rec.ensure(has_rec ? (size_t)np * sizeof(DevPrimRec) : 16));
 
     LAY_TRY(hipMemsetAsync(d_words, 0, 16 * sizeof(uint32_t), st));
     LAY_TRY(hipMemsetAsync(d_last, 0, np, st));
@@ -176,7 +182,8 @@
     pa.spheres = s->spheres.as<DevSphere>();
     pa.mat_kind = d_mat_kind;
     pa.n_triangles = s->n_triangles;
-    k_prims<<<blocks(np, kThreads), kThreads, 0, st>>>(pa, order, d_last, np, s->n_triangles + s->n_spheres, s->tris.as<uint4>(), s->prim_shade.as<uint4>(), has_attr ? s->prim_attr.as<uint4>() : nullptr);
+    k_prims<<<blocks(np, kThreads), kThreads, 0, st>>>(pa, order, d_last, np, s->n_triangles + s->n_spheres, s->tris.as<uint4>(), s->prim_shade.as<uint4>(), has_attr ? s->prim_attr.as<uint4>() : nullptr,
+                                                               has_rec ? s->prim_rec.as<uint4>() : nullptr);
     LAY_TRY(hipGetLastError());
     uint32_t words[16];
     if (wide) {
@@ -199,7 +206,7 @@
         LAY_TRY(s->nodes4.ensure(16));
     }
 #undef LAY_TRY
-    set_record_layout(s, n_interior, n4, words[2], words[3], np, has_attr, root_leaf ? (YK_LEAF_BIT | tree.root_words[6]) : 0u, wide && s->upd.opt.wide_bvh == 2);
+    set_record_layout(s, n_interior, n4, words[2], words[3], np, has_attr, has_rec, root_leaf ? (YK_LEAF_BIT | tree.root_words[6]) : 0u, wide && s->upd.opt.wide_bvh == 2);
     return YK_LAYOUT_REASON_NONE;
 }
 
diff --git a/yuki_amd/csrc/yk_scene_records.cpp b/yuki_amd/csrc/yk_scene_records.cpp
--- a/yuki_amd/csrc/yk_scene_records.cpp
+++ b/yuki_amd/csrc/yk_scene_records.cpp
@@ -4,6 +4,7 @@
 #include <cstring>
 
 #include "yk_kernels.h"
+#include "yk_scene_layout.h"
 
 using namespace yk;
 
@@ -175,10 +176,25 @@
     }
 }
 
+static void layout_prim_rec(const HostLayoutInput& in, SceneRecords& out) {
+    if (in.opt.shade_records == 0) return;
+    static_assert(sizeof(DevPrimRec) == sizeof(uint4[8]), "DevPrimRec is eight 16-byte words");
+    const size_t np = out.prim_shade.size();
+    out.prim_rec.resize(np);
+    for (size_t p = 0; p < np; ++p) {
+        uint4 tri[3], attr[4] = {}, rec[8];
+        std::memcpy(tri, &out.tris[3 * p], sizeof(tri));
+        if (!out.prim_attr.empty()) std::memcpy(attr, &out.prim_attr[4 * p], sizeof(attr));
+        lay::prim_rec_words(tri, out.prim_shade[p], attr, rec);
+        std::memcpy(&out.prim_rec[p], rec, sizeof(rec));
+    }
+}
+
 SceneRecords layout_records_host(const HostLayoutInput& in) {
     SceneRecords out;
     layout_nodes(in, out);
     layout_wide(in, out);
     layout_prims(in, out);
+    layout_prim_rec(in, out);
     return out;
 }
diff --git a/yuki_amd/csrc/yk_scene_records.h b/yuki_amd/csrc/yk_scene_records.h
--- a/yuki_amd/csrc/yk_scene_records.h
+++ b/yuki_amd/csrc/yk_scene_records.h
@@ -6,7 +6,7 @@
 #include "yk_host.h"
 
 struct LayoutOptions {
-    int64_t top_nodes = 0, wide_bvh = 0;
+    int64_t top_nodes = 0, wide_bvh = 0, shade_records = 0;
 };
 
 struct HostLayoutInput {
@@ -29,6 +29,7 @@
     std::vector<float4> tris;
     std::vector<uint4> prim_shade;
     std::vector<float4> prim_attr;
+    std::vector<yk::DevPrimRec> prim_rec;
     uint32_t root_ref = 0;
     bool wide_auto = false;
 };
```

After: 2303 Mray/s (median of 6 runs). About the same (+0.5%).
